# Healthcare-Robotics/mr-gan

Measured on AMD Instinct MI355X. Metric: GAN train steps/sec (labeled+unlabeled+G) at batch 4096, higher is better.
Workload: dtype bf16; 1 GPU; BASELINE configs[1]: synthetic N=65536 x D=512, K=6, batch 4096 per GPU, labeled 100/class; one step = D sub-step (3B rows) + G sub-step (2B rows) + both Adam updates; global_batch=4096, rows_per_gpu=4096, parallelism=single, batch_statistics=n/a, launch=hipGraph replay

## Files before the change

include/mrgan_abi.h:

```cpp
#ifndef MRGAN_ABI_H
#define MRGAN_ABI_H

#include <stddef.h>
#include <stdint.h>

#ifdef __cplusplus
extern "C" {
#endif

typedef struct mrgan_handle mrgan_handle;
typedef void* mrgan_stream;

enum { MRGAN_F32 = 0, MRGAN_BF16 = 1, MRGAN_FP8 = 2 };
enum { MRGAN_NET_G = 0, MRGAN_NET_D = 1 };
enum {
    MRGAN_FLAG_SYNC_STATS = 1,
    MRGAN_FLAG_FLAT_GRADS = 2,
    MRGAN_FLAG_GRAPH      = 4,
    MRGAN_FLAG_GRAD_BF16  = 8,
    MRGAN_FLAG_GAUSS_NOISE = 16
};

#define MRGAN_MAX_CLASSES 32
#define MRGAN_MAX_MODELS 16
// ... 25 lines not shown

int mrgan_select_model(mrgan_handle* h, int model);

int mrgan_num_tensors(const mrgan_handle* h, int net, int* n);
int mrgan_tensor_shape(const mrgan_handle* h, int net, int idx, int* rows, int* cols);
int mrgan_set_weights(mrgan_handle* h, int net, int idx, const float* src_dev, mrgan_stream stream);
int mrgan_get_weights(mrgan_handle* h, int net, int idx, float* dst_dev, mrgan_stream stream);
int mrgan_get_slot(mrgan_handle* h, int net, int idx, int which, float* dst_dev, mrgan_stream stream);
int mrgan_set_slot(mrgan_handle* h, int net, int idx, int which, const float* src_dev, mrgan_stream stream);
int mrgan_get_iterations(mrgan_handle* h, mrgan_stream stream, uint32_t* iterations_host);
int mrgan_set_iterations(mrgan_handle* h, uint32_t iterations, uint32_t batch_counter, mrgan_stream stream);

typedef struct mrgan_disc_args {
    const float* x_lab_dev; const int32_t* idx_lab_dev; const int32_t* labels_dev;
    const float* x_unl_dev; const int32_t* idx_unl_dev;
    const float* z_dev;
    int64_t ld_x_lab, ld_x_unl;
    int32_t stream_mode, reserved;
} mrgan_disc_args;

typedef struct mrgan_gen_args {
    const float* x_unl_dev; const int32_t* idx_unl_dev;
    const float* z_dev;
    int64_t ld_x_unl;
    int32_t stream_mode, reserved;
} mrgan_gen_args;

enum { MRGAN_D_GEN = 0, MRGAN_D_MAIN = 1, MRGAN_D_ADAM = 2, MRGAN_D_NPHASES = 3 };
enum { MRGAN_G_GEN = 0, MRGAN_G_FEAT = 1, MRGAN_G_BWD = 2, MRGAN_G_TAIL = 3, MRGAN_G_ADAM = 4, MRGAN_G_NPHASES = 5 };
int mrgan_disc_step(mrgan_handle* h, const mrgan_disc_args* a, int phase_first, int phase_last,
                    float* out3_host, mrgan_stream stream);
int mrgan_gen_step(mrgan_handle* h, const mrgan_gen_args* a, int phase_first, int phase_last,
                   float* out1_host, mrgan_stream stream);
enum { MRGAN_FP8_DRY_PASSES = 5 };
enum { MRGAN_FP8_CAL_QUERY = 0, MRGAN_FP8_CAL_BEGIN = 1, MRGAN_FP8_CAL_END_PASS = 2, MRGAN_FP8_CAL_DONE = 3 };
int mrgan_fp8_calibration(mrgan_handle* h, int kind, int action, mrgan_stream stream);

typedef struct mrgan_sup_args {
    const float* x_dev; const int32_t* idx_dev; const int32_t* labels_dev;
    int64_t ld_x;
    int32_t stream_mode, rows_valid;
} mrgan_sup_args;
int mrgan_sup_step(mrgan_handle* h, const mrgan_sup_args* a, float* out2_host, mrgan_stream stream);
typedef struct mrgan_sup_group_args {
    const float* x_dev; const int32_t* idx_dev; const int32_t* labels_dev;
    int64_t ld_x;
    int64_t x_model_stride, idx_model_stride, labels_model_stride;
    int32_t stream_mode, rows_valid;
} mrgan_sup_group_args;
int mrgan_sup_step_group(mrgan_handle* h, const mrgan_sup_group_args* a, float* out2_host, mrgan_stream stream);

int32_t mrgan_logmel_frames(int64_t n_samples);
int mrgan_logmel(const float* y_dev, int64_t n_trials, int64_t n_samples, int64_t ld_y, int32_t sr, int32_t n_mels,
                 float* out_dev, int64_t ld_out, mrgan_stream stream);

int mrgan_train_pair(mrgan_handle* h, const mrgan_disc_args* d, const mrgan_gen_args* g, mrgan_stream stream);
int mrgan_pair_hint(mrgan_handle* h, int on);

typedef struct mrgan_disc_group_args {
    const float* x_lab_dev; const int32_t* idx_lab_dev; const int32_t* labels_dev;
    const float* x_unl_dev; const int32_t* idx_unl_dev;
    const float* z_dev;
    int64_t ld_x_lab, ld_x_unl;
    int64_t x_lab_model_stride, idx_lab_model_stride, labels_model_stride;
    int64_t x_unl_model_stride, idx_unl_model_stride, z_model_stride;
    int32_t stream_mode, reserved;
} mrgan_disc_group_args;
typedef struct mrgan_gen_group_args {
    const float* x_unl_dev; const int32_t* idx_unl_dev;
    const float* z_dev;
    int64_t ld_x_unl;
    int64_t x_unl_model_stride, idx_unl_model_stride, z_model_stride;
    int32_t stream_mode, reserved;
} mrgan_gen_group_args;
int mrgan_disc_step_group(mrgan_handle* h, const mrgan_disc_group_args* a, float* out3_host, mrgan_stream stream);
int mrgan_gen_step_group(mrgan_handle* h, const mrgan_gen_group_args* a, float* out1_host, mrgan_stream stream);
int mrgan_train_pair_group(mrgan_handle* h, const mrgan_disc_group_args* d, const mrgan_gen_group_args* g, mrgan_stream stream);

enum {
    MRGAN_TUNE_CHAIN = 0,
    MRGAN_TUNE_KC_CFG = 1,
    MRGAN_TUNE_KS_GROUP = 4,
    MRGAN_TUNE_PAIR_GEN = 5,
    MRGAN_TUNE_HEAD_MFMA = 6
};
int mrgan_set_tuning(mrgan_handle* h, int knob, int value);

enum {
    MRGAN_REGION_BN_STATS = 0,
    MRGAN_REGION_FM_MOMENTS = 1,
    MRGAN_REGION_BN_BWD = 2,
    MRGAN_REGION_GRAD_D = 3,
    MRGAN_REGION_GRAD_G = 4,
    MRGAN_REGION_WORKSPACE = 5,
    MRGAN_REGION_GRAD_D_BF16 = 6,
    MRGAN_REGION_GRAD_G_BF16 = 7,
    MRGAN_REGION_TAIL_D = 8,
    MRGAN_REGION_TAIL_G = 9
};
int mrgan_region(mrgan_handle* h, int region, void** ptr_dev, size_t* bytes);

int mrgan_eval_error(mrgan_handle* h, const float* x_dev, const int32_t* idx_dev, int64_t ld_x,
                     const int32_t* labels_dev, int64_t n, float* err_host, mrgan_stream stream);
int mrgan_predict_logits(mrgan_handle* h, const float* x_dev, const int32_t* idx_dev, int64_t ld_x, int64_t n,
                         float* logits_dev, mrgan_stream stream);

enum { MRGAN_SAL_LOGIT = 0, MRGAN_SAL_XENT = 1, MRGAN_SAL_MSE = 2 };
enum { MRGAN_SAL_RAW = 0, MRGAN_SAL_HEATMAP = 1 };
typedef struct mrgan_saliency_args {
    const float* x_dev; const int32_t* idx_dev; int64_t ld_x; int64_t n;
    const int32_t* targets_dev;
    int32_t objective;
    int32_t post;
    float* out_dev; int64_t ld_out;
    int32_t* classes_out_dev;
} mrgan_saliency_args;
int mrgan_input_gradient(mrgan_handle* h, const mrgan_saliency_args* a, mrgan_stream stream);

enum { MRGAN_ATTR_NOISE = 0, MRGAN_ATTR_PATH = 1 };
enum { MRGAN_ATTR_MAX_DRAWS = 4096, MRGAN_ATTR_NOISE_SEG = 255 };
typedef struct mrgan_attribution_args {
    const float* x_dev; const int32_t* idx_dev; int64_t ld_x; int64_t n;
    const int32_t* targets_dev;
    int32_t objective;
    int32_t post;
    float* out_dev; int64_t ld_out;
    int32_t* classes_out_dev;
    int32_t method;
    int32_t draws;
    float sigma_input, sigma_hidden;
    const float* baseline_dev;
    int32_t multiply;
    int32_t reserved;
} mrgan_attribution_args;
int mrgan_attribution(mrgan_handle* h, const mrgan_attribution_args* a, mrgan_stream stream);

int mrgan_read_metrics(mrgan_handle* h, float* out8_host, int reset, mrgan_stream stream);

enum { MRGAN_PROF_NAME_LEN = 96 };
int mrgan_profile_begin(mrgan_handle* h);
int mrgan_profile_end(mrgan_handle* h, mrgan_stream stream, int max_kernels, char* names, float* ms, int32_t* launches,
                      double* flops, double* bytes, int* n_kernels);

#ifdef __cplusplus
}
#endif
#endif
```

include/mrgan_debug.h:

```cpp
#ifndef MRGAN_DEBUG_H
#define MRGAN_DEBUG_H

#include "mrgan_abi.h"

#ifdef __cplusplus
extern "C" {
#endif

int mrgan_debug_noise(mrgan_handle* h, uint32_t site, uint32_t seg, uint32_t step, uint32_t row0, int rows, int cols,
                      float* out_dev, mrgan_stream stream);
int mrgan_debug_tr_probe(uint16_t* out1024_dev, mrgan_stream stream);
int mrgan_debug_ablate(mrgan_handle* h, int bits);
int mrgan_debug_buffer(mrgan_handle* h, int kind, int l, void** ptr_dev, int* rows_per_seg, int* ld, int* elem_size);
int mrgan_debug_gemm_time(int op, int m, int n, int k, int nbatch, int splits, int reps, int ablate, int kc_cfg, float* avg_us);

typedef struct mrgan_debug_gemm_desc {
    int32_t dtype, op, m, n, k, nbatch, splits;
    int32_t kchunk;
    int32_t kc_cfg;
    int32_t tune_bits;
    int32_t seg_stride, seg_rows;
    const void* a; int64_t a_bs, a_si, a_sk;
    const void* b; int64_t b_bs, b_sk, b_sj;
    int32_t act, n_valid;
    const float* bias;
    void* out; int64_t out_bs; int32_t ldo;
    float sigma; uint32_t site, seg0; int32_t seg_step; uint32_t iter_step, row0;
    uint32_t iter;
    uint64_t seed;
    uint16_t* mask; int64_t mask_bs; int32_t ldm;
    const void* h; int64_t h_bs; int32_t ldh;
    int32_t cs_mode; float* cs1; float* cs2; int32_t ldcs;
    const float* bn_mu; const float* bn_rstd;
    float* slab; int64_t slab_stride;
    void* q8; int64_t q8_bs; int32_t ldq8;
    void* q8t; int64_t q8t_bs; int32_t ldq8t;
    const void* slot_a; const void* slot_b; void* slot_o;
    int32_t gauss;
} mrgan_debug_gemm_desc;
typedef struct mrgan_debug_fold { const float* src; float* dst; int64_t stride; int32_t nsrc, n, ngroups; } mrgan_debug_fold;
int mrgan_debug_gemm_launch(const mrgan_debug_gemm_desc* d, int count, int grouped, const mrgan_debug_fold* fold,
                            char* kname, int kname_len, mrgan_stream stream);

int mrgan_debug_gemm_fp8(int m, int n, int k, const float* a_dev, const float* b_dev, const float* bias_dev, int act, float scale_a,
                         float scale_b, float* out_dev, int reps, float* avg_us, int kc_cfg, mrgan_stream stream);

int mrgan_debug_quant8(const void* src, int64_t src_bs, int ld, int rows, int cols, int nb, int prow, void* dst, int64_t dst_bs, int ldd,
                       void* dstt, int64_t dstt_bs, int lddt, void* slot_dev, int fmt, mrgan_stream stream);
int mrgan_debug_fp8_update_scales(void* slots_dev, int n, mrgan_stream stream);


typedef struct mrgan_debug_stage_seg {
    const float* src; const int32_t* idx; int64_t ld;
    int32_t rows, cols, cols_pad;
    void* out; int32_t ldo;
    float sigma; uint32_t site, seg;
    int32_t gen, stream; uint32_t iter_off;
    int32_t models; int64_t src_ms, idx_ms, out_ms;
} mrgan_debug_stage_seg;
typedef struct mrgan_debug_stage_desc {
    int32_t dtype;
    mrgan_debug_stage_seg s[5]; int32_t nseg;
    uint64_t seed; uint32_t row0;
    uint32_t iter, batch;
    int32_t gauss;
} mrgan_debug_stage_desc;
int mrgan_debug_stage(const mrgan_debug_stage_desc* d, mrgan_stream stream);

int mrgan_debug_reduce_partials(const float* src, int nsrc, int64_t stride, int n, int ngroups, float* dst, int models,
                                int64_t model_stride, mrgan_stream stream);
int mrgan_debug_colsum_finalize(const float* part1, const float* part2, int npart, int ld, int n, float* out, int nseg,
                                mrgan_stream stream);

typedef struct mrgan_debug_bn_apply_desc {
    int32_t dtype;
    const void* h; void* out; int32_t ld, rows, cols;
    const float* cs1; const float* cs2; int32_t npart, ldcs;
    float count, eps;
    const float* gamma; const float* beta;
    float* mu; float* rstd;
    int64_t cs_seg_stride;
    int32_t nseg; int64_t seg_rows;
} mrgan_debug_bn_apply_desc;
int mrgan_debug_bn_apply(const mrgan_debug_bn_apply_desc* d, mrgan_stream stream);

typedef struct mrgan_debug_bn_bwd_desc {
    int32_t dtype;
    const void* dy; const void* h; void* dpre; int32_t ld, rows, cols;
    const float* cs1; const float* cs2; int32_t npart, ldcs;
    float count;
    const float* gamma; const float* mu; const float* rstd;
    float* db_part;
} mrgan_debug_bn_bwd_desc;
int mrgan_debug_bn_bwd(const mrgan_debug_bn_bwd_desc* d, mrgan_stream stream);

typedef struct mrgan_debug_head_desc {
    int32_t dtype;
    const void* f; int64_t f_bs; int32_t ldf;
    int32_t rows, nseg, seg_kind[3];
    int32_t feat, feat_valid, classes;
    const float* w; int32_t ldw; const float* b;
    const int32_t* labels; int32_t labels_stream; uint32_t batch;
    float inv_count, unl_weight;
    float* logits; int64_t logits_bs;
    void* dpre; int64_t dpre_bs; int32_t ldd;
    float* part; int64_t part_stride; int32_t off_db, off_dbf;
    float* loss_part;
    int32_t models; int64_t model_stride, labels_ms;
    int32_t* err_count;
    void* q8; int64_t q8_bs; int32_t ldq8;
    void* q8t; int64_t q8t_bs; int32_t ldq8t;
    void* q8_slot;
} mrgan_debug_head_desc;
int mrgan_debug_head(const mrgan_debug_head_desc* d, mrgan_stream stream);

typedef struct mrgan_debug_head_wide_desc {
    mrgan_debug_head_desc h;
    const uint16_t* mask; int64_t mask_bs; int32_t ldm;
    void* w6c; void* w6r;
} mrgan_debug_head_wide_desc;
int mrgan_debug_head_wide(const mrgan_debug_head_wide_desc* d, mrgan_stream stream);

typedef struct mrgan_debug_fm_desc {
    int32_t dtype;
    const float* cs; int32_t npart_fake, npart_real, ldcs;
    float count, grad_scale; int32_t feat, feat_valid;
    const uint16_t* mask; int32_t ldm;
    void* dpre; int32_t ldd; int32_t rows;
    float* loss_out; float* accum;
    void* q8; int32_t ldq8; void* q8_slot;
    float* lscratch; uint32_t* lcount;
} mrgan_debug_fm_desc;
int mrgan_debug_fm(const mrgan_debug_fm_desc* d, mrgan_stream stream);

typedef struct mrgan_debug_chain_op {
    int32_t K, N, n_valid;
    const void* W; const float* bias;
    float sigma; uint32_t site;
    void* out; int64_t out_bs; int32_t ldo;
    uint16_t* mask; int64_t mask_bs; int32_t ldm;
    float* cs; int32_t ldcs;
} mrgan_debug_chain_op;
typedef struct mrgan_debug_chain_desc {
    int32_t variant;
    mrgan_debug_chain_op fwd[3], dx[3];
    int32_t rows, nseg, block_rows;
    int32_t models; int64_t model_stride;
    const void* a; int64_t a_bs; int32_t lda, a_cols;
    int32_t seg0; uint64_t seed; uint32_t row0; int32_t gauss;
    uint32_t iter, batch;
    mrgan_debug_head_desc head;
    mrgan_debug_fm_desc fm; const void* fm_feat; int32_t fm_ldf;
} mrgan_debug_chain_desc;
int mrgan_debug_chain(const mrgan_debug_chain_desc* d, char* kname, int kname_len, mrgan_stream stream);

typedef struct mrgan_debug_adam_tile {
    float* p; float* m; float* v;
    const float* g; int32_t nslab; int64_t slab_stride;
    float* flat; void* flat16;
    void* w16; void* wt16;
    void* w8; void* w8t; void* w8_slot;
    int32_t ld, ldt, rows, cols;
} mrgan_debug_adam_tile;
typedef struct mrgan_debug_adam_desc {
    const mrgan_debug_adam_tile* tiles; int32_t ntiles, mode;
    float b1, b2, eps;
    uint32_t iter, batch; float lr_t;
    const float* loss_part; int32_t nloss_part; float inv_rows; float* step_out; float* accum;
    float* flat_tail;
    int32_t publish_next, advance_batch; float lr;
    int32_t models; int64_t model_stride;
} mrgan_debug_adam_desc;
int mrgan_debug_adam(const mrgan_debug_adam_desc* d, uint32_t next_out[4], mrgan_stream stream);

#ifdef __cplusplus
}
#endif
// ... 2 lines not shown
```

mr_gan_amd/csrc/aux_kernels.h:

```cpp
#pragma once
#include "common.h"

namespace mrgan {

constexpr int KMAX = 8;
constexpr int KWIDE = 32;
constexpr int class_pitch(int classes) { return classes <= KMAX ? KMAX : KWIDE; }
constexpr int HEAD_ROWS = 32;
constexpr int HEAD_CHUNK = 256;

struct StageSeg {
    const float* src; const int32_t* idx; long ld;
    int rows, cols, cols_pad;
    void* out; int ldo;
    float sigma; uint32_t site, seg;
    int gen;
    int stream;
    uint32_t iter_off;
    int models; long src_ms, idx_ms, out_ms;
};
struct StageArgs {
    StageSeg s[5]; int nseg;
    uint64_t seed; uint32_t row0;
    const DevState* cur;
    int gauss;
    int ry; uint32_t ry_mul;
};
int launch_stage(int bf16, const StageArgs& a, hipStream_t s);

struct BnApplyArgs {
    const void* h; void* out; int ld; int rows; int cols;
    const float* cs1; const float* cs2; int npart; int ldcs;
    float count, eps;
    const float* gamma; const float* beta;
    float* mu; float* rstd;
    long cs_seg_stride;
    int nseg; long seg_rows;
    int models; long model_stride; uint32_t seg_mul;
};
int launch_bn_apply(int bf16, const BnApplyArgs& a, hipStream_t s);

struct BnBwdArgs {
    const void* dy; const void* h; void* dpre; int ld; int rows; int cols;
    const float* cs1; const float* cs2; int npart; int ldcs;
    float count;
    const float* gamma; const float* mu; const float* rstd;
    float* db_part;
    int models; long model_stride;
};
int launch_bn_bwd(int bf16, const BnBwdArgs& a, hipStream_t s);
int stat_row_blocks(int rows);

enum { HEAD_LAB = 0, HEAD_UNL = 1, HEAD_FAKE = 2, HEAD_EVAL = 3, HEAD_LOGITS = 4,
       HEAD_MSE = 5,
       HEAD_SAL_LOGIT = 6, HEAD_SAL_XENT = 7, HEAD_SAL_MSE = 8 };
struct HeadArgs {
    const void* f; long f_bs; int ldf;
    int rows, nseg, seg_kind[3];
    int feat, feat_valid, classes;
    const float* w; int ldw; const float* b;
    const int32_t* labels;
    const DevState* st; int labels_stream;
    float inv_count, unl_weight;
    float* logits; long logits_bs;
    void* dpre; long dpre_bs; int ldd;
    float* part; long part_stride;
    int off_db, off_dbf;
    float* loss_part;
    int models; long model_stride, labels_ms;
    union {
        int* err_count;
        int32_t* classes_out;
    };
    unsigned char* q8; long q8_bs; int ldq8;
    unsigned char* q8t; long q8t_bs; int ldq8t;
    Fp8Slot* q8_slot;
};
int launch_head(int bf16, const HeadArgs& a, hipStream_t s);
int launch_reduce_partials(const float* src, int nsrc, long stride, int n, int ngroups, float* dst, hipStream_t s, int models = 1,
                           long model_stride = 0);
int init_kernel_attributes();

enum { SAL_RAW = 0, SAL_HEATMAP = 1 };
struct SaliencyFinishArgs {
    const void* g; int ldg;
    int rows, cols;
    float* out; long ldo;
    int mode;
};
int launch_saliency_finish(int bf16, const SaliencyFinishArgs& a, hipStream_t s);

struct PathStageArgs {
    const float* src; const int32_t* idx; long ld;
    const float* baseline;
    float alpha;
    int rows, cols, cols_pad;
    void* out; int ldo;
};
int launch_path_stage(int bf16, const PathStageArgs& a, hipStream_t s);
struct AttrAccumArgs {
    const void* g; int ldg;
    int rows, cols;
    float* out; long ldo;
    int mode;
    int draw, draws;
    int multiply;
    const float* x; const int32_t* idx; long ld_x;
    const float* baseline;
};
int launch_attr_accum(int bf16, const AttrAccumArgs& a, hipStream_t s);

struct FmArgs {
    const float* cs; int npart_fake, npart_real, ldcs;
    float count, grad_scale; int feat, feat_valid;
    const uint16_t* mask; int ldm;
    void* dpre; int ldd; int rows;
    float* loss_out; float* accum;
    unsigned char* q8; int ldq8; Fp8Slot* q8_slot;
    int rb;
    float* lscratch; unsigned int* lcount;
    int models; long model_stride;
};
int launch_fm(int bf16, const FmArgs& a, hipStream_t s);

int launch_colsum_finalize(const float* part1, const float* part2, int npart, int ld, int n, float* out , hipStream_t s,
                           int nseg = 1 );

struct AdamTile {
    float* p; float* m; float* v;
    const float* g; int nslab; long slab_stride;
    float* flat;
    __bf16* flat16;
    __bf16* w16; __bf16* wt16;
    unsigned char* w8; unsigned char* w8t; Fp8Slot* w8_slot;
// ... 20 lines not shown
```

mr_gan_amd/csrc/aux_kernels.hip:

```cpp
#include "aux_kernels.h"
#include "head.h"

namespace mrgan {
namespace {

template <typename T> __device__ __forceinline__ void load8(const T* p, float v[8]);
template <> __device__ __forceinline__ void load8<float>(const float* p, float v[8]) {
    const f32x4 a = *(const f32x4*)p, b = *(const f32x4*)(p + 4);
#pragma unroll
    for (int i = 0; i < 4; ++i) { v[i] = a[i]; v[4 + i] = b[i]; }
}
template <> __device__ __forceinline__ void load8<__bf16>(const __bf16* p, float v[8]) {
    const bf16x8 a = *(const bf16x8*)p;
#pragma unroll
    for (int i = 0; i < 8; ++i) v[i] = (float)a[i];
}
template <typename T> __device__ __forceinline__ void store8(T* p, const float v[8]);
template <> __device__ __forceinline__ void store8<float>(float* p, const float v[8]) {
    f32x4 a, b;
#pragma unroll
    for (int i = 0; i < 4; ++i) { a[i] = v[i]; b[i] = v[4 + i]; }
    *(f32x4*)p = a; *(f32x4*)(p + 4) = b;
}
template <> __device__ __forceinline__ void store8<__bf16>(__bf16* p, const float v[8]) {
// ... 21 lines not shown
    const float* const xsrc = sg.src + (long)model * sg.src_ms;
    const int32_t* const xidx = sg.idx ? sg.idx + (long)model * sg.idx_ms : nullptr;
    const bool noisy = sg.gen || sg.sigma > 0.f;
    const float sigs = (sg.gen ? 1.0f : sg.sigma) * (GAUSS ? 1.0f : NOISE_SCALE);
    const int cg = (lane & 15) * 8, rl = lane >> 4;
    const int col = cbase + cg;
    const bool vec_ok = !sg.gen && (sg.ld & 3) == 0 && ((uintptr_t)xsrc & 15) == 0 && col + 7 < sg.cols;
    long srow[8];
#pragma unroll
    for (int it = 0; it < 8; ++it) {
        const int row = rbase + it * 4 + rl;
        srow[it] = (!sg.gen && row < sg.rows) ? (xidx ? (long)xidx[o + row] : (o + row)) : 0;
    }
    float v[8][8];
#pragma unroll
    for (int it = 0; it < 8; ++it) {
#pragma unroll
        for (int c = 0; c < 8; ++c) v[it][c] = 0.f;
        const int row = rbase + it * 4 + rl;
        if (!sg.gen && row < sg.rows) {
            const float* src = xsrc + srow[it] * sg.ld + col;
            if (vec_ok) load8<float>(src, v[it]);
            else {
#pragma unroll
                for (int c = 0; c < 8; ++c) if (col + c < sg.cols) v[it][c] = src[c];
            }
        }
    }
    if constexpr (GAUSS) {
        if (noisy) {
            const uint32_t ph = gauss_pairhash(noise_key(seed, sg.site * 256u + sg.seg, st.iter + sg.iter_off), a.row0 + (uint32_t)rbase, lane);
#pragma unroll
            for (int cb = 0; cb < 4; ++cb) {
                const int c0 = cbase + cb * 32;
                if (c0 >= sg.cols) break;
                const f32x16 nz = gauss_block(ph, (uint32_t)(c0 + lc), lane);
#pragma unroll
                for (int r = 0; r < 16; ++r) glds[wave][acc_row(r, lh)][lc] = nz[r];
                __builtin_amdgcn_fence(__ATOMIC_RELEASE, "wavefront");
                __builtin_amdgcn_wave_barrier();
                if ((cg >> 5) == cb) {
#pragma unroll
                    for (int it = 0; it < 8; ++it) {
                        const f32x4 n0 = *(const f32x4*)&glds[wave][it * 4 + rl][cg & 31], n1 = *(const f32x4*)&glds[wave][it * 4 + rl][(cg & 31) + 4];
#pragma unroll
                        for (int c = 0; c < 4; ++c) {
                            if (col + c < sg.cols) v[it][c] = fmaf(sigs, n0[c], v[it][c]);
                            if (col + 4 + c < sg.cols) v[it][4 + c] = fmaf(sigs, n1[c], v[it][4 + c]);
                        }
                    }
                }
                __builtin_amdgcn_fence(__ATOMIC_ACQ_REL, "wavefront");
                __builtin_amdgcn_wave_barrier();
            }
        }
    } else if (noisy) {
        const uint32_t rowhash = noise_rowhash(noise_key(seed, sg.site * 256u + sg.seg, st.iter + sg.iter_off), a.row0 + (uint32_t)(rbase + lc));
        const i32x4 hfrag = hadamard_frag(lane);
#pragma unroll
        for (int cb = 0; cb < 4; ++cb) {
            const int c0 = cbase + cb * 32;
            if (c0 >= sg.cols) break;
            const i32x16 nz = noise_block(rowhash, (uint32_t)c0 >> 5, lane, hfrag);
#pragma unroll
            for (int r = 0; r < 16; ++r) nlds[wave][acc_row(r, lh)][cb * 32 + lc] = (short)nz[r];
        }
        __builtin_amdgcn_fence(__ATOMIC_RELEASE, "wavefront");
        __builtin_amdgcn_wave_barrier();
    }
    if (col >= sg.cols_pad) return;
#pragma unroll
    for (int it = 0; it < 8; ++it) {
        const int rr = it * 4 + rl, row = rbase + rr;
        if (row >= sg.rows) break;
        if (!GAUSS && noisy && col < sg.cols) {
            const s16x8 nz = *(const s16x8*)&nlds[wave][rr][cg];
#pragma unroll
            for (int c = 0; c < 8; ++c) if (col + c < sg.cols) v[it][c] = fmaf(sigs, (float)nz[c], v[it][c]);
        }
        store8<T>(out + (long)row * sg.ldo + col, v[it]);
    }
}

constexpr int RB = 64, CB = 64;

__device__ __forceinline__ void fold_partials(const float* part, int npart, int ldcs, int col0, int ncols, float (*scr)[CB], float* out) {
    const int t = threadIdx.x, cq = (t & 15) * 4, pl = t >> 4;
    f32x4 s0 = {0.f, 0.f, 0.f, 0.f}, s1 = s0;
    if (col0 + cq < ncols) {
        int p = pl;
        for (; p + 16 < npart; p += 32) {
            s0 += *(const f32x4*)(part + (long)p * ldcs + col0 + cq);
            s1 += *(const f32x4*)(part + (long)(p + 16) * ldcs + col0 + cq);
        }
        for (; p < npart; p += 16) s0 += *(const f32x4*)(part + (long)p * ldcs + col0 + cq);
    }
    s0 += s1;
    *(f32x4*)(&scr[pl][cq]) = s0;
    __syncthreads();
    if (t < CB) {
        float s = 0.f;
#pragma unroll
        for (int k = 0; k < 16; ++k) s += scr[k][t];
        out[t] = s;
    }
    __syncthreads();
}

template <typename T>
__global__ __launch_bounds__(256) void bn_apply_kernel(const BnApplyArgs a) {
    __shared__ float sc[CB], sh[CB];
    __shared__ float scr[16][CB], f1[CB], f2[CB];
    const int t = threadIdx.x, col0 = blockIdx.x * CB;
    const int model = (int)((blockIdx.z * a.seg_mul) >> 16), seg = (int)blockIdx.z - model * a.nseg;
    const long moff = (long)model * a.model_stride;
    const float* const gamma = (const float*)((const char*)a.gamma + moff);
    const float* const beta = (const float*)((const char*)a.beta + moff);
    float* const mu = (float*)((char*)a.mu + moff);
    float* const rstd_out = (float*)((char*)a.rstd + moff);
    fold_partials((const float*)((const char*)a.cs1 + moff) + (long)seg * a.cs_seg_stride, a.npart, a.ldcs, col0, a.ld, scr, f1);
    fold_partials((const float*)((const char*)a.cs2 + moff) + (long)seg * a.cs_seg_stride, a.npart, a.ldcs, col0, a.ld, scr, f2);
    if (t < CB) {
        const int col = col0 + t;
        float scale = 0.f, shift = 0.f;
        if (col < a.ld) {
            const float mean = f1[t] / a.count;
            const float var = fmaxf(f2[t] / a.count - mean * mean, 0.f);
            const float rstd = 1.0f / sqrtf(var + a.eps);
            if (col < a.cols) { scale = gamma[col] * rstd; shift = beta[col] - mean * scale; }
            if (blockIdx.y == 0) { mu[(long)seg * a.ld + col] = mean; rstd_out[(long)seg * a.ld + col] = rstd; }
        }
        sc[t] = scale; sh[t] = shift;
    }
    __syncthreads();
    const int cg = t & 7, rl = t >> 3, c0 = col0 + cg * 8;
    if (c0 >= a.ld) return;
    const T* h = (const T*)((const char*)a.h + moff) + (long)seg * a.seg_rows * a.ld;
    T* out = (T*)((char*)a.out + moff) + (long)seg * a.seg_rows * a.ld;
    const int r1 = min(a.rows, (int)(blockIdx.y + 1) * RB);
    for (int r = blockIdx.y * RB + rl; r < r1; r += 32) {
        float v[8];
        load8<T>(h + (long)r * a.ld + c0, v);
#pragma unroll
        for (int i = 0; i < 8; ++i) v[i] = v[i] * sc[cg * 8 + i] + sh[cg * 8 + i];
        store8<T>(out + (long)r * a.ld + c0, v);
    }
}

template <typename T>
__global__ __launch_bounds__(256) void bn_bwd_kernel(const BnBwdArgs a) {
    __shared__ float cA[CB], cB[CB], cM[CB], cR[CB], cG[CB];
    __shared__ float red[32][CB];
    const int t = threadIdx.x, col0 = blockIdx.x * CB;
    const long moff = (long)blockIdx.z * a.model_stride;
    fold_partials((const float*)((const char*)a.cs1 + moff), a.npart, a.ldcs, col0, a.ld, red, cB);
    fold_partials((const float*)((const char*)a.cs2 + moff), a.npart, a.ldcs, col0, a.ld, red, cG);
    if (t < CB) {
        const int col = col0 + t;
        float g = 0.f, mu = 0.f, rs = 0.f;
        if (col < a.cols) {
            g = ((const float*)((const char*)a.gamma + moff))[col]; mu = ((const float*)((const char*)a.mu + moff))[col];
            rs = ((const float*)((const char*)a.rstd + moff))[col];
        }
        cA[t] = g * rs / a.count; cM[t] = mu; cR[t] = rs;
    }
    __syncthreads();
    const int cg = t & 7, rl = t >> 3, c0 = col0 + cg * 8;
    float acc[8];
#pragma unroll
    for (int i = 0; i < 8; ++i) acc[i] = 0.f;
    if (c0 < a.ld) {
        const T* dy = (const T*)((const char*)a.dy + moff);
        const T* h = (const T*)((const char*)a.h + moff);
        T* dpre = (T*)((char*)a.dpre + moff);
        const int r1 = min(a.rows, (int)(blockIdx.y + 1) * RB);
        for (int r = blockIdx.y * RB + rl; r < r1; r += 32) {
            float hv[8], d[8], o[8];
            load8<T>(h + (long)r * a.ld + c0, hv);
            load8<T>(dy + (long)r * a.ld + c0, d);
#pragma unroll
            for (int i = 0; i < 8; ++i) {
                const int c = cg * 8 + i;
                const float xh = (hv[i] - cM[c]) * cR[c];
                const float dh = cA[c] * (a.count * d[i] - cB[c] - xh * cG[c]);
                o[i] = dh * (-expm1f(-hv[i]));
                acc[i] += o[i];
            }
            store8<T>(dpre + (long)r * a.ld + c0, o);
        }
    }
#pragma unroll
    for (int i = 0; i < 8; ++i) red[rl][cg * 8 + i] = acc[i];
    __syncthreads();
    if (t < CB && col0 + t < a.ld) {
        float s = 0.f;
#pragma unroll
        for (int k = 0; k < 32; ++k) s += red[k][t];
        ((float*)((char*)a.db_part + moff))[(long)blockIdx.y * a.ld + col0 + t] = s;
    }
}

constexpr int HR = HEAD_ROWS;
template <bool WIDE> struct HeadAcc { typedef float type; };
#ifndef MRGAN_HEAD_ACC_F32
template <> struct HeadAcc<true> { typedef double type; };
#endif
__device__ __forceinline__ float head_fma(float a, float b, float c) { return fmaf(a, b, c); }
__device__ __forceinline__ double head_fma(float a, float b, double c) { return fma((double)a, (double)b, c); }
template <typename T, bool Q8 = false, int KP = KMAX, bool SAL = false>
__global__ __launch_bounds__(256) void head_kernel(const HeadArgs a) {
    constexpr int KG = KP / 4;
    typedef typename HeadAcc<(KP > KMAX && sizeof(T) == 2)>::type acc_t;
    extern __shared__ __attribute__((aligned(16))) float hl[];
    const int CH = min(a.feat, HEAD_CHUNK), nch = (a.feat + CH - 1) / CH;
    const int LDF = CH + 8;
    float* f_lds = hl;
    float* w_lds = f_lds + HR * LDF;
    float* dl_lds = w_lds + CH * KP;
    float* red = dl_lds + HR * KP;

    const int t = threadIdx.x, lane = t & 63, wave = t >> 6;
    const int seg = blockIdx.y, kind = a.seg_kind[seg];
    const int row_blk = blockIdx.x * HR;
    const int blk = seg * gridDim.x + blockIdx.x;
    const long moff = (long)blockIdx.z * a.model_stride;
    const T* f = (const T*)((const char*)a.f + moff) + (long)seg * a.f_bs;
    const float* const w6 = (const float*)((const char*)a.w + moff);

    const int cpr = CH / 8;
    auto load_chunk = [&](int c0) {
        for (int ci = t; ci < HR * cpr; ci += 256) {
            const int r = ci / cpr, c = (ci - r * cpr) * 8;
            float v[8] = {0.f, 0.f, 0.f, 0.f, 0.f, 0.f, 0.f, 0.f};
            if (row_blk + r < a.rows && c0 + c < a.feat) load8<T>(f + (long)(row_blk + r) * a.ldf + c0 + c, v);
            *(f32x4*)(f_lds + r * LDF + c) = (f32x4){v[0], v[1], v[2], v[3]};
            *(f32x4*)(f_lds + r * LDF + c + 4) = (f32x4){v[4], v[5], v[6], v[7]};
        }
        for (int k = t; k < CH; k += 256) {
            f32x4 w[KG];
#pragma unroll
            for (int g = 0; g < KG; ++g) w[g] = (f32x4){0.f, 0.f, 0.f, 0.f};
            if (c0 + k < a.feat_valid) {
#pragma unroll
                for (int g = 0; g < KG; ++g) w[g] = *(const f32x4*)(w6 + (long)(c0 + k) * a.ldw + 4 * g);
            }
#pragma unroll
            for (int c = 0; c < 4; ++c)
#pragma unroll
                for (int g = 0; g < KG; ++g) if (c + 4 * g >= a.classes) w[g][c] = 0.f;
#pragma unroll
            for (int g = 0; g < KG; ++g) *(f32x4*)(w_lds + k * KP + 4 * g) = w[g];
        }
    };

    constexpr int LPR = 256 / HR;
    const int r = t / LPR, part = t % LPR;
    acc_t la[KP];
#pragma unroll
    for (int c = 0; c < KP; ++c) la[c] = 0.f;
    for (int ch = 0; ch < nch; ++ch) {
        if (ch) __syncthreads();
        load_chunk(ch * CH);
        __syncthreads();
        for (int kk = 0; kk < CH / LPR; ++kk) {
            const int k = kk * LPR + part;
            const float fv = f_lds[r * LDF + k];
            f32x4 w[KG];
#pragma unroll
            for (int g = 0; g < KG; ++g) w[g] = *(const f32x4*)(w_lds + k * KP + 4 * g);
// ... 756 lines not shown
```

mr_gan_amd/csrc/engine.hip:

```cpp
#include "engine_internal.h"

namespace mrgan {
thread_local LaunchTimer g_launch_timer = {nullptr, nullptr, 0, 0};
}

namespace {

int prof_cat(mrgan_handle* h, const char* name) {
    for (size_t i = 0; i < h->prof_names.size(); ++i)
        if (h->prof_names[i] == name) return (int)i;
    h->prof_names.push_back(name);
    return (int)h->prof_names.size() - 1;
}
__global__ void prof_delay_kernel(int us) {
    for (int i = 0; i < us; ++i) __builtin_amdgcn_s_sleep(36);
}


void prof_backlog(mrgan_handle* h, hipStream_t s) {
    if (!h->prof) return;
    hipLaunchKernelGGL(prof_delay_kernel, dim3(1), dim3(64), 0, s, 400);
}
void prof_arm(mrgan_handle* h) {
    if (!h->prof) return;
// ... 77 lines not shown
              int ldd, unsigned char* dstt, long dstt_bs, int lddt, int slot, int fmt, hipStream_t s) {
    Quant8Args q;
    memset(&q, 0, sizeof q);
    q.src = (const __bf16*)src; q.src_bs = src_bs; q.ld = ld; q.rows = rows; q.cols = cols; q.prow = prow; q.nb = nb;
    q.dst = dst; q.dst_bs = dst_bs; q.ldd = ldd; q.dstt = dstt; q.dstt_bs = dstt_bs; q.lddt = lddt;
    q.slot = h->slots + slot; q.fmt = fmt;
    PROFB("quant8_kernel", launch_quant8(q, s), (double)nb * prow * cols * (2.0 + (dst ? 1.0 : 0.0) + (dstt ? 1.0 : 0.0)));
    return 0;
}
int fp8_quant_images(mrgan_handle* h, const void* src, int width, int nb, unsigned char* img, unsigned char* imgt, int ldt, int slot,
                     int fmt, hipStream_t s) {
    const long bs = (long)h->S * width;
    return fp8_quant(h, src, bs, width, h->B, width, (int)round_up(h->B, 64), nb, img, bs, width, imgt, h->S, ldt, slot, fmt, s);
}

int dense_fwd(mrgan_handle* h, const Dense& L, int kind, const void* x, int rows, int nb, void* out, int act, const NoiseSite& nz,
              const ReluMask& m, const ColSums& cs, hipStream_t s, const Fp8Use& f8 = NO_FP8, const DrawKey* dk = nullptr) {
    const Fp8Images& q = L.q;
    const bool fp8 = q.on && kind != KIND_EVAL;
    const long a_bs = (long)h->S * L.Kp;
    if (fp8 && f8.quant_in)
        CHK(fp8_quant_images(h, x, L.Kp, nb, x8_view(h, L), f8.wgrad ? x8t_view(h, L) : nullptr, q.ldxt, q.sx[kind], FP8_E4M3, s));
    GemmArgs g = with_handle(h, fp8       ? gemm_fwd_args(rows, L.Kp, L.Np, nb, x8_view(h, L), a_bs, L.Kp, q.w8t, L.Kp, true)
                                : h->bf16 ? gemm_fwd_args(rows, L.Kp, L.Np, nb, x, a_bs, L.Kp, L.W->wt16, L.Kp, true)
                                          : gemm_fwd_args(rows, L.Kp, L.Np, nb, x, a_bs, L.Kp, L.W->p, L.Np, false));
    Epi& e = g.e;
    e.act = act; e.n_valid = L.N; e.bias = L.b->p;
    if (kind == KIND_EVAL) {
        e.st = nullptr;
        if (dk) { e.st = dk->st; e.seed = dk->seed; e.row0 = dk->row0; }
        g.B = selected(h, g.B); e.bias = selected(h, e.bias);
    }
    e.out = out; e.out_bs = (long)h->S * L.Np; e.ldo = L.Np;
    e.sigma = nz.sigma; e.site = nz.site; e.seg0 = nz.seg0; e.seg_step = nz.seg_step; e.iter_step = nz.iter_step;
    epi_mask(h, e, m);
    epi_sums(e, cs, L.Np);
    if (fp8) {
        e.qa = h->slots + q.sx[kind]; e.qb = h->slots + q.sw;
        if (f8.to && f8.to->q.on) epi_images(h, e, f8.to->q.x8, f8.wgrad ? f8.to->q.x8t : nullptr, L.Np, f8.to->q.ldxt, f8.to->q.sx[kind]);
    }
    return run_gemm(h, EPI_FWD, g, 2.0 * rows * nb * L.K * L.N, dense_bytes(h, (double)rows * nb, L), s);
}

int dense_dx(mrgan_handle* h, const Dense& L, int kind, const void* dy, int rows, int nb, void* out, int act, int n_valid,
             const ReluMask& m, const void* hprev, const ColSums& cs, hipStream_t s, const Fp8Use& f8 = NO_FP8) {
    const Fp8Images& q = L.q;
    const long a_bs = (long)h->S * L.Np;
    if (q.on && f8.quant_in)
        CHK(fp8_quant_images(h, dy, L.Np, nb, q.g8, f8.wgrad ? q.g8t : nullptr, q.ldgt, q.sg[kind], FP8_E5M2, s));
    GemmArgs g = with_handle(h, q.on ? gemm_dx_args(rows, L.Kp, L.Np, nb, q.g8, a_bs, L.Np, q.w8, L.Np)
                                     : gemm_dx_args(rows, L.Kp, L.Np, nb, dy, a_bs, L.Np,
                                                    h->bf16 ? (const void*)L.W->w16 : (const void*)L.W->p, L.Np));
    Epi& e = g.e;
    e.act = act; e.n_valid = n_valid;
    if (kind == KIND_EVAL) g.B = selected(h, g.B);
    e.out = out; e.out_bs = (long)h->S * L.Kp; e.ldo = L.Kp;
    epi_mask(h, e, m);
    e.h = hprev; e.h_bs = (long)h->S * L.Kp; e.ldh = L.Kp;
    epi_sums(e, cs, L.Kp);
    e.bn_mu = h->bn_mu; e.bn_rstd = h->bn_rstd;
    if (q.on) {
        e.qa = h->slots + q.sg[kind]; e.qb = h->slots + q.sw;
        if (f8.to && f8.to->q.on) epi_images(h, e, f8.to->q.g8, f8.wgrad ? f8.to->q.g8t : nullptr, L.Kp, f8.to->q.ldgt, f8.to->q.sg[kind]);
    }
    return run_gemm(h, EPI_DX, g, 2.0 * rows * nb * L.K * L.N, dense_bytes(h, (double)rows * nb, L), s);
}

double dw_args(mrgan_handle* h, GemmArgs& g, const Dense& L, int kind, const void* x, const void* dy, int rows, int nseg) {
    const bool dense = h->bf16 != 0;
    const int vrows = dense ? nseg * h->S : (nseg - 1) * h->S + rows;
    if (L.q.on) {
        g = with_handle(h, gemm_dw_args(L.Kp, L.Np, vrows, L.splits, vrows / L.splits, 0, 0, x8t_view(h, L), L.q.ldxt, L.q.g8t, L.q.ldgt,
                                        true, L.slabs));
        g.e.qa = h->slots + L.q.sx[kind]; g.e.qb = h->slots + L.q.sg[kind];
    } else {
        g = with_handle(h, gemm_dw_args(L.Kp, L.Np, vrows, L.splits, gemm_dw_kchunk(vrows, L.splits), h->S, dense ? h->S : rows,
                                        x, L.Kp, dy, L.Np, false, L.slabs));
    }
    return 2.0 * rows * nseg * L.K * L.N;
}

struct DwJob { const Dense* L; const void* x; const void* dy; };

int dense_dw_all(mrgan_handle* h, int kind, const DwJob* jobs, int n, int rows, int nseg, hipStream_t s, const FoldJob* fold = nullptr) {
    GemmArgs gs[KS_GROUP_MAX];
    DwJob js[KS_GROUP_MAX];
    double fl[KS_GROUP_MAX], total = 0.0, bytes = 0.0;
    if (n > KS_GROUP_MAX) return fail(-1, "dense_dw_all: too many products");
    std::copy(jobs, jobs + n, js);
    const int ngroup = (int)(std::stable_partition(js, js + n, [](const DwJob& j) { return !j.L->q.on; }) - js);
    for (int i = 0; i < n; ++i) fl[i] = dw_args(h, gs[i], *js[i].L, kind, js[i].x, js[i].dy, rows, nseg);
    for (int i = 0; i < ngroup; ++i) { total += fl[i] * h->grouped; bytes += dw_bytes(h, (double)rows * nseg, *js[i].L) * h->grouped; }
    int first = 0;
    if (h->bf16 && ngroup > 0) {
        const char* kname = "gemm";
        prof_arm(h);
        const int r = launch_gemm_bf16_dw_group(gs, ngroup, s, &kname, fold);
        prof_done(h, kname, total, bytes);
        if (r < 0) return fail(r, "grouped weight-gradient launch failed");
        if (r == 0) { first = ngroup; fold = nullptr; }
    }
    for (int i = first; i < n; ++i) CHK(run_gemm(h, EPI_SLAB, gs[i], fl[i], dw_bytes(h, (double)rows * nseg, *js[i].L), s));
    if (fold) PROF("reduce_partials_kernel", launch_reduce_partials(fold->src, fold->nsrc, fold->stride, fold->n, fold->ngroups, fold->dst, s,
                                                                    h->grouped, fold->model_stride));
    return 0;
}

}
int mrgan::fp8_update_scales(mrgan_handle* h, hipStream_t s) {
    PROF("fp8_update_scales_kernel", launch_fp8_update_scales(h->slots, FP8_NSLOT, s));
    return 0;
}
int mrgan::fp8_refresh_weights(mrgan_handle* h, int net, hipStream_t s) {
    int n;
    const Dense* Ls = net_layers(h, net, &n);
    for (int l = 0; l < n; ++l) {
        const Dense& L = Ls[l];
        if (L.q.on) CHK(fp8_quant(h, L.W->w16, 0, L.Np, L.Kp, L.Np, L.Kp, 1, L.q.w8, 0, L.Np, L.q.w8t, 0, L.Kp, L.q.sw, FP8_E4M3, s));
    }
    return 0;
}
namespace {

int run_adam(mrgan_handle* h, int net, int mode, bool with_metrics, hipStream_t s, int advance_batch = 0) {
    AdamArgs a;
    memset(&a, 0, sizeof a);
    if (mode != ADAM_REDUCE_ONLY) { a.next = h->state + (h->cur ^ 1); a.advance_batch = advance_batch; a.lr = h->cfg.lr; }
    a.tiles = net == MRGAN_NET_D ? h->tiles_d_dev : h->tiles_g_dev;
    a.ntiles = net == MRGAN_NET_D ? h->ntiles_d : h->ntiles_g;
    a.mode = mode; a.b1 = h->cfg.beta1; a.b2 = h->cfg.beta2; a.eps = h->cfg.adam_eps;
    a.st = h->state + h->cur;
    if (with_metrics) {
        a.loss_part = h->loss_part; a.nloss_part = h->head_nblk; a.inv_rows = 1.0f / (float)h->Bg;
        a.step_out = h->step_out; a.accum = h->accum;
        a.flat_tail = h->flat_d + h->flat_d_n;
    }
    a.models = h->grouped; a.model_stride = (long)h->W;
    {
        const std::vector<Tensor>& ts = net == MRGAN_NET_D ? h->dt : h->gt;
        double bytes = 0.0;
        for (const Tensor& t : ts) bytes += (double)t.prow * t.pcol * (24.0 + 4.0 * std::max(1, t.nslab) + (t.w16 ? 4.0 : 0.0));
        PROFB("adam_kernel", launch_adam(a, s), bytes);
    }
    return 0;
}

int gen_fwd_head(mrgan_handle* h, int nb, hipStream_t s) {
    CHK(dense_fwd(h, h->g[0], KIND_D, h->zbuf, h->B, nb, h->h1, ACT_SOFTPLUS, NO_NOISE, NO_MASK, ColSums{CS_SUM_SQ, h->cs_bn1, h->cs_bn2}, s));
    if (h->sync_stats) {
        const int n = h->g[0].Np;
        PROF("colsum_finalize_kernel", launch_colsum_finalize(h->cs_bn1, h->cs_bn2, h->tiles_m, n, n, h->r_bn_stats, s, nb));
    }
    return 0;
}
int gen_fwd_tail(mrgan_handle* h, int nb, int fake_seg_slot, uint32_t fake_seg_id, hipStream_t s) {
    const int n = h->g[0].Np;
    BnApplyArgs b;
    memset(&b, 0, sizeof b);
    b.h = h->h1; b.out = h->hbn; b.ld = n; b.rows = h->B; b.cols = h->g[0].N;
    b.nseg = nb; b.seg_rows = h->S;
    if (h->sync_stats) { b.cs1 = h->r_bn_stats; b.cs2 = h->r_bn_stats + n; b.npart = 1; b.cs_seg_stride = 2 * n; }
    else { b.cs1 = h->cs_bn1; b.cs2 = h->cs_bn2; b.npart = h->tiles_m; b.cs_seg_stride = (long)h->tiles_m * n; }
    b.ldcs = n; b.count = h->stat_count; b.eps = h->cfg.bn_eps;
    b.gamma = h->gt[2].p; b.beta = h->gt[3].p; b.mu = h->bn_mu; b.rstd = h->bn_rstd;
    b.models = h->grouped; b.model_stride = (long)h->W;
    PROF("bn_apply_kernel", launch_bn_apply(h->bf16, b, s));
    CHK(dense_fwd(h, h->g[1], KIND_D, h->hbn, h->B, nb, h->h2, ACT_SOFTPLUS, NO_NOISE, NO_MASK, NO_SUMS, s, Fp8Use{nullptr, true, true}));
    void* out = rowptr(h, h->xin[0], (long)fake_seg_slot * h->S, h->Dp);
    const NoiseSite nz = {h->cfg.sigma[0], 0, fake_seg_id, nb > 1 ? -(int)fake_seg_id : 1, nb > 1 ? 1u : 0u};
    CHK(dense_fwd(h, h->g[2], KIND_D, h->h2, h->B, nb, out, ACT_LINEAR, nz, NO_MASK, NO_SUMS, s));
    return 0;
}

int disc_fwd_train(mrgan_handle* h, int kind, int nb, bool fm_sums, int x0_slot, hipStream_t s, int l_end = 5) {
    for (int l = 0; l < l_end; ++l) {
        const void* in = l == 0 ? rowptr(h, h->xin[0], (long)x0_slot * h->S, h->Dp) : h->xin[l];
        void* out = l < 4 ? h->xin[l + 1] : h->feat;
        const NoiseSite nz = {l < 4 ? h->cfg.sigma[l + 1] : 0.f, (uint32_t)(l + 1), 0, 1, 0};
        const bool last = l == 4;
        CHK(dense_fwd(h, h->d[l], kind, in, h->B, nb, out, ACT_RELU, nz, relu_mask(h, l), ColSums{(last && fm_sums) ? CS_SUM : CS_NONE, h->cs_f, nullptr},
                      s, Fp8Use{last ? nullptr : &h->d[l + 1], kind == KIND_D, l == 0}));
    }
// ... 212 lines not shown

int gen_chain_fwd(mrgan_handle* h, hipStream_t s) {
    ChainArgs c = chain_args(h, CH_V_GFWD, 2, chain_block_rows(h, 2));
    for (int i = 0; i < 3; ++i) c.fwd[i] = chain_fwd_op(h, 2 + i, i == 2);
    return run_chain(h, c, chain_flops(h, c, false), s);
}

int fm_grad(mrgan_handle* h, hipStream_t s) {
    FmArgs f;
    memset(&f, 0, sizeof f);
    if (h->sync_stats) { f.cs = h->r_fm; f.npart_fake = 1; f.npart_real = 1; }
    else { f.cs = h->cs_f; f.npart_fake = f.npart_real = fm_parts(h); }
    f.ldcs = h->Fp; f.count = h->stat_count; f.grad_scale = h->fm_scale; f.feat = h->Fp; f.feat_valid = h->F;
    f.mask = h->mask[4]; f.ldm = h->ldm[4]; f.dpre = h->dpre[4]; f.ldd = h->Fp; f.rows = h->B;
    f.loss_out = h->step_out + 3; f.accum = h->accum + 3;
    f.lscratch = h->fm_scratch; f.lcount = h->fm_count;
    f.models = h->grouped; f.model_stride = (long)h->W;
    if (h->fp8) { f.dpre = nullptr; f.q8 = h->d[4].q.g8; f.ldq8 = h->Fp; f.q8_slot = h->slots + h->d[4].q.sg[KIND_G]; }
    if (!h->use_chain) {
        PROF("fm_kernel", launch_fm(h->bf16, f, s));
        return 0;
    }
    ChainArgs c = chain_args(h, CH_V_GBWD, 1, chain_block_rows(h, 1));
    c.fm = f; c.fm_feat = (const __bf16*)h->feat; c.fm_ldf = h->Fp;
    for (int i = 0; i < 3; ++i) c.dx[i] = chain_dx_op(h, 4 - i, false);
    return run_chain(h, c, chain_flops(h, c, false), s);
}

int disc_dx_to_input(mrgan_handle* h, hipStream_t s) {
    for (int l = h->use_chain ? 1 : 4; l >= 1; --l)
        CHK(dense_dx(h, h->d[l], KIND_G, h->dpre[l], h->B, 1, h->dpre[l - 1], ACT_RELU, h->d[l - 1].N, relu_mask(h, l - 1), nullptr,
                     NO_SUMS, s, Fp8Use{&h->d[l - 1], false, false}));
    return dense_dx(h, h->d[0], KIND_G, h->dpre[0], h->B, 1, h->dxfake, ACT_LINEAR, h->cfg.d_in, NO_MASK, nullptr,
                    ColSums{CS_SUM, h->cs_db3g, nullptr}, s);
}

int gen_phase(mrgan_handle* h, const mrgan_gen_args* a, int phase, hipStream_t s) {
    const int B = h->B, tm = h->tiles_m, N1p = h->g[0].Np;
    if (phase == MRGAN_G_GEN) {
        prof_backlog(h, s);
        StageArgs st;
        memset(&st, 0, sizeof st);
        const bool ready = h->gen_ready && !a->z_dev;
        h->gen_ready = ready ? 1 : 0;
        h->xbase = ready ? 3 : 0;
        set_gen_view(h, ready ? 1 : 0);
        const bool staged = ready && h->real_staged;
        h->real_staged = 0;
        if (!staged) {
            data_seg(st.s[0], h, a->x_unl_dev, a->idx_unl_dev, a->ld_x_unl, h->xbase + 1, 1, a->stream_mode, h->gs.x_unl, h->gs.idx_unl);
            st.nseg = 1;
            stage_common(st, h, a->z_dev, a->stream_mode, ready ? -1 : 1);
            PROF("stage_kernel", launch_stage(h->bf16, st, s));
        }
        if (!ready) CHK(gen_fwd_head(h, 1, s));
    } else if (phase == MRGAN_G_FEAT) {
        if (!h->gen_ready) CHK(gen_fwd_tail(h, 1, 0, 0, s));
        h->gen_ready = 0;
        CHK(disc_fwd_train(h, 1, 2, true, h->xbase, s, h->use_chain ? 2 : 5));
        if (h->use_chain) CHK(gen_chain_fwd(h, s));
        if (h->sync_stats) {
            const int np = fm_parts(h);
            PROF("colsum_finalize_kernel", launch_colsum_finalize(h->cs_f, h->cs_f + (size_t)np * h->Fp, np, h->Fp, h->Fp, h->r_fm, s));
        }
    } else if (phase == MRGAN_G_BWD) {
        CHK(fm_grad(h, s));
        CHK(disc_dx_to_input(h, s));
        CHK(dense_dx(h, h->g[2], KIND_G, h->dxfake, B, 1, h->dpre2g, ACT_SOFTPLUS, h->g[1].N, NO_MASK, h->h2,
                     ColSums{CS_SUM, h->cs_db2g, nullptr}, s));
        CHK(dense_dx(h, h->g[1], KIND_G, h->dpre2g, B, 1, h->dhbn, ACT_LINEAR, h->g[0].N, NO_MASK, h->h1,
                     ColSums{CS_SUM_XHAT, h->cs_dbeta, h->cs_dgamma}, s, Fp8Use{nullptr, true, true}));
        if (h->sync_stats) {
            PROF("colsum_finalize_kernel", launch_colsum_finalize(h->cs_dbeta, h->cs_dgamma, tm, N1p, N1p, h->r_bn_bwd, s));
        }
    } else if (phase == MRGAN_G_TAIL) {
        BnBwdArgs b;
        memset(&b, 0, sizeof b);
        b.dy = h->dhbn; b.h = h->h1; b.dpre = h->dpre1g; b.ld = N1p; b.rows = B; b.cols = h->g[0].N;
        if (h->sync_stats) { b.cs1 = h->r_bn_bwd; b.cs2 = h->r_bn_bwd + N1p; b.npart = 1; }
        else { b.cs1 = h->cs_dbeta; b.cs2 = h->cs_dgamma; b.npart = tm; }
        b.ldcs = N1p; b.count = h->stat_count; b.gamma = h->gt[2].p; b.mu = h->bn_mu; b.rstd = h->bn_rstd;
        b.db_part = h->db1g_part;
        b.models = h->grouped; b.model_stride = (long)h->W;
        PROF("bn_bwd_kernel", launch_bn_bwd(h->bf16, b, s));
        const DwJob jobs[3] = {{&h->g[2], h->h2, h->dxfake}, {&h->g[0], h->zbuf, h->dpre1g}, {&h->g[1], h->hbn, h->dpre2g}};
        CHK(dense_dw_all(h, KIND_G, jobs, 3, B, 1, s));
        if (h->flat_grads) CHK(run_adam(h, MRGAN_NET_G, ADAM_REDUCE_ONLY, false, s));
    } else if (phase == MRGAN_G_ADAM) {
        CHK(run_adam(h, MRGAN_NET_G, h->flat_grads ? ADAM_FROM_FLAT : ADAM_FUSED, false, s, a->stream_mode ? 1 : 0));
        if (h->fp8) CHK(fp8_update_scales(h, s));
        h->cur ^= 1;
    }
    return 0;
}

int sup_step(mrgan_handle* h, const mrgan_sup_args* a, hipStream_t s) {
    const int B = h->B;
    prof_backlog(h, s);
    StageArgs st;
    memset(&st, 0, sizeof st);
    data_seg(st.s[0], h, a->x_dev, a->idx_dev, a->ld_x, 0, 0, a->stream_mode, h->gs.x_lab, h->gs.idx_lab);
    st.nseg = 1;
    stage_common(st, h, nullptr, 0, -1);
    PROF("stage_kernel", launch_stage(h->bf16, st, s));
    CHK(disc_fwd_train(h, 0, 1, false, 0, s, 5));
    HeadArgs hd = head_args(h, {HEAD_MSE}, B, true);
    hd.labels = a->labels_dev; hd.labels_stream = a->stream_mode;
    hd.inv_count = 1.0f / (float)(a->rows_valid > 0 ? a->rows_valid : B); hd.unl_weight = 0.f;
    PROF("head_kernel", launch_head(h->bf16, hd, s));
    h->head_nblk = 3 * ceil_div(B, HEAD_ROWS);
    CHK(disc_bwd(h, 1, 4, ceil_div(B, HEAD_ROWS), s));
    CHK(run_adam(h, MRGAN_NET_D, ADAM_FUSED, true, s, a->stream_mode ? 1 : 0));
    h->cur ^= 1;
    return 0;
}

int check_disc_args(const mrgan_handle* h, const mrgan_disc_args* a) {
    if (!a || !a->x_lab_dev || !a->x_unl_dev || !a->labels_dev) return fail(-2, "disc_step: x_lab, x_unl and labels are required");
    if (a->ld_x_lab < h->cfg.d_in || a->ld_x_unl < h->cfg.d_in) return fail(-2, "disc_step: row pitch smaller than d_in");
    return 0;
}
int check_gen_args(const mrgan_handle* h, const mrgan_gen_args* a) {
    if (!a || !a->x_unl_dev) return fail(-2, "gen_step: x_unl is required");
    if (a->ld_x_unl < h->cfg.d_in) return fail(-2, "gen_step: row pitch smaller than d_in");
    return 0;
}
int check_sup_args(const mrgan_handle* h, const mrgan_sup_args& a, const char* entry) {
    if (a.ld_x < h->cfg.d_in) return fail(-2, "%s: row pitch smaller than d_in", entry);
    if (h->flat_grads || h->cfg.world != 1) return fail(-3, "%s: single-GPU handles only", entry);
    if (h->fp8) return fail(-3, "%s: the fp8 mode covers the GAN step only", entry);
    if (a.rows_valid < 0 || a.rows_valid > h->B) return fail(-2, "%s: rows_valid outside [0, batch]", entry);
    if (a.rows_valid && a.stream_mode) return fail(-2, "%s: a short batch cannot be combined with stream mode", entry);
    return 0;
}

struct GroupScope {
    mrgan_handle* h;
    GroupScope(mrgan_handle* h_, const mrgan_handle::GroupStrides& gs) : h(h_) { h->grouped = h->models; h->gs = gs; h->pair_gen = 0; h->pair_g = nullptr; }
    ~GroupScope() { h->grouped = 1; memset(&h->gs, 0, sizeof h->gs); }
};
mrgan_disc_args single_args(const mrgan_disc_group_args* a) {
    mrgan_disc_args d;
    memset(&d, 0, sizeof d);
    d.x_lab_dev = a->x_lab_dev; d.idx_lab_dev = a->idx_lab_dev; d.labels_dev = a->labels_dev;
    d.x_unl_dev = a->x_unl_dev; d.idx_unl_dev = a->idx_unl_dev; d.z_dev = a->z_dev;
    d.ld_x_lab = a->ld_x_lab; d.ld_x_unl = a->ld_x_unl; d.stream_mode = a->stream_mode;
    return d;
}
mrgan_gen_args single_args(const mrgan_gen_group_args* a) {
    mrgan_gen_args g;
    memset(&g, 0, sizeof g);
    g.x_unl_dev = a->x_unl_dev; g.idx_unl_dev = a->idx_unl_dev; g.z_dev = a->z_dev; g.ld_x_unl = a->ld_x_unl; g.stream_mode = a->stream_mode;
    return g;
}
mrgan_sup_args single_args(const mrgan_sup_group_args* a) {
    mrgan_sup_args u;
    memset(&u, 0, sizeof u);
    u.x_dev = a->x_dev; u.idx_dev = a->idx_dev; u.labels_dev = a->labels_dev; u.ld_x = a->ld_x;
    u.stream_mode = a->stream_mode; u.rows_valid = a->rows_valid;
    return u;
}
int sup_step_group(mrgan_handle* h, const mrgan_sup_group_args* a, hipStream_t s) {
    GroupScope scope(h, {(long)a->x_model_stride, (long)a->idx_model_stride, (long)a->labels_model_stride, 0, 0, 0});
    const mrgan_sup_args u = single_args(a);
    return sup_step(h, &u, s);
}
int disc_step_group(mrgan_handle* h, const mrgan_disc_group_args* a, hipStream_t s) {
    GroupScope scope(h, {(long)a->x_lab_model_stride, (long)a->idx_lab_model_stride, (long)a->labels_model_stride,
                         (long)a->x_unl_model_stride, (long)a->idx_unl_model_stride, (long)a->z_model_stride});
// ... 479 lines not shown
```

mr_gan_amd/csrc/engine_debug.hip:

```cpp
#include "engine_internal.h"

namespace mrgan {
int launch_tr_probe(unsigned short* out, hipStream_t s);
}

namespace {

template <typename T>
__global__ void to_f32_kernel(const T* src, long lds, float* dst, long ldd, int rows, int cols) {
    const int c = blockIdx.x * 64 + (threadIdx.x & 63), r = blockIdx.y * 4 + (threadIdx.x >> 6);
    if (r >= rows || c >= cols) return;
    dst[(long)r * ldd + c] = Elem<T>::to_f32(src[(long)r * lds + c]);
}

}

extern "C" {

int mrgan_debug_noise(mrgan_handle* h, uint32_t site, uint32_t seg, uint32_t step, uint32_t row0, int rows, int cols, float* out,
                      mrgan_stream stream) {
    if (!h || !out) return fail(-1, "null argument");
    if (h->gauss && (row0 & 1u)) return fail(-1, "debug_noise: a true-Gaussian handle draws row pairs, row0 must be even");
    CHK(launch_noise_debug(h->gauss, h->cfg.seed, site, seg, step, row0, rows, cols, out, (hipStream_t)stream));
    return 0;
// ... 309 lines not shown
}

int mrgan_debug_stage(const mrgan_debug_stage_desc* d, mrgan_stream stream) {
    if (!d || d->nseg < 1 || d->nseg > 5) return fail(-1, "debug_stage: 1 .. 5 segments");
    if (d->dtype != MRGAN_F32 && d->dtype != MRGAN_BF16) return fail(-1, "debug_stage: dtype must be fp32 or bf16");
    if (d->gauss && (d->row0 & 1u)) return fail(-1, "debug_stage: the true-Gaussian generator draws row pairs, row0 must be even");
    StageArgs a;
    memset(&a, 0, sizeof a);
    for (int i = 0; i < d->nseg; ++i) {
        const mrgan_debug_stage_seg& g = d->s[i];
        StageSeg& o = a.s[i];
        if (!g.out || g.rows < 1 || g.cols < 1 || (!g.gen && !g.src)) return fail(-1, "debug_stage: segment %d: null argument", i);
        if (g.cols_pad < g.cols || (g.cols_pad % 8) || g.ldo < g.cols_pad || (g.ldo % 8) || !al(g.out, 16) || (g.out_ms % 16))
            return fail(-1, "debug_stage: segment %d: rows of out are stored 8 elements at a time (out, out_ms, ldo %% 8, cols <= cols_pad <= ldo, cols_pad %% 8)", i);
        if (!g.gen && g.ld < g.cols) return fail(-1, "debug_stage: segment %d: ld >= cols", i);
        o.src = g.src; o.idx = g.idx; o.ld = g.ld; o.rows = g.rows; o.cols = g.cols; o.cols_pad = g.cols_pad;
        o.out = g.out; o.ldo = g.ldo; o.sigma = g.sigma; o.site = g.site; o.seg = g.seg; o.gen = g.gen; o.stream = g.stream;
        o.iter_off = g.iter_off; o.models = g.models; o.src_ms = g.src_ms; o.idx_ms = g.idx_ms; o.out_ms = g.out_ms;
    }
    a.nseg = d->nseg; a.seed = d->seed; a.row0 = d->row0; a.gauss = d->gauss;
    DevState* st = nullptr;
    if (int r = debug_devstate(d->iter, d->batch, 0.f, &st)) return r;
    a.cur = st;
    hipStream_t s = (hipStream_t)stream;
    const int r = debug_finish("debug_stage", launch_stage(d->dtype == MRGAN_BF16, a, s), s);
    hipFree(st);
    return r;
}

int mrgan_debug_reduce_partials(const float* src, int nsrc, int64_t stride, int n, int ngroups, float* dst, int models, int64_t model_stride,
                                mrgan_stream stream) {
    if (!src || !dst || nsrc < 1 || n < 1 || ngroups < 1 || models < 1) return fail(-1, "debug_reduce_partials: empty problem");
    if (stride < n) return fail(-1, "debug_reduce_partials: stride >= n");
    if (model_stride % 4) return fail(-1, "debug_reduce_partials: model_stride counts bytes of whole floats");
    hipStream_t s = (hipStream_t)stream;
    return debug_finish("debug_reduce_partials", launch_reduce_partials(src, nsrc, stride, n, ngroups, dst, s, models, model_stride), s);
}

int mrgan_debug_colsum_finalize(const float* part1, const float* part2, int npart, int ld, int n, float* out, int nseg, mrgan_stream stream) {
    if (!part1 || !part2 || !out || npart < 1 || n < 1 || nseg < 1) return fail(-1, "debug_colsum_finalize: empty problem");
    if (!al(part1, 16) || !al(part2, 16) || (ld % 4)) return fail(-1, "debug_colsum_finalize: partial rows are read 16 bytes at a time (pointers, ld %% 4)");
    if (ld < n) return fail(-1, "debug_colsum_finalize: ld >= n");
    hipStream_t s = (hipStream_t)stream;
    return debug_finish("debug_colsum_finalize", launch_colsum_finalize(part1, part2, npart, ld, n, out, s, nseg), s);
}

static int debug_cs_check(const char* who, const float* cs1, const float* cs2, int npart, int ldcs, int width) {
    if (!cs1 || !cs2 || npart < 1) return fail(-1, "%s: column partial sums missing", who);
    if (!al(cs1, 16) || !al(cs2, 16) || (ldcs % 4)) return fail(-1, "%s: partial sums are read 16 bytes at a time (pointers, ldcs %% 4)", who);
    if (ldcs < width) return fail(-1, "%s: ldcs must hold the %d columns the kernel folds", who, width);
    return 0;
}

int mrgan_debug_bn_apply(const mrgan_debug_bn_apply_desc* d, mrgan_stream stream) {
    if (!d || !d->h || !d->out || !d->gamma || !d->beta || !d->mu || !d->rstd || d->rows < 1 || d->cols < 1) return fail(-1, "debug_bn_apply: null argument");
    if (d->dtype != MRGAN_F32 && d->dtype != MRGAN_BF16) return fail(-1, "debug_bn_apply: dtype must be fp32 or bf16");
    if (int r = debug_cs_check("debug_bn_apply", d->cs1, d->cs2, d->npart, d->ldcs, d->ld)) return r;
    if (d->ld < d->cols || (d->ld % 8) || !al(d->h, 16) || !al(d->out, 16)) return fail(-1, "debug_bn_apply: ld >= cols, ld %% 8 == 0 and 16-byte aligned h / out");
    if (d->nseg > 1 && ((d->cs_seg_stride % 4) || d->seg_rows < d->rows)) return fail(-1, "debug_bn_apply: cs_seg_stride %% 4 == 0 and seg_rows >= rows");
    BnApplyArgs a;
    memset(&a, 0, sizeof a);
    a.h = d->h; a.out = d->out; a.ld = d->ld; a.rows = d->rows; a.cols = d->cols;
    a.cs1 = d->cs1; a.cs2 = d->cs2; a.npart = d->npart; a.ldcs = d->ldcs; a.count = d->count; a.eps = d->eps;
    a.gamma = d->gamma; a.beta = d->beta; a.mu = d->mu; a.rstd = d->rstd;
    a.cs_seg_stride = d->cs_seg_stride; a.nseg = d->nseg; a.seg_rows = d->seg_rows;
    hipStream_t s = (hipStream_t)stream;
    return debug_finish("debug_bn_apply", launch_bn_apply(d->dtype == MRGAN_BF16, a, s), s);
}

int mrgan_debug_bn_bwd(const mrgan_debug_bn_bwd_desc* d, mrgan_stream stream) {
    if (!d || !d->dy || !d->h || !d->dpre || !d->gamma || !d->mu || !d->rstd || !d->db_part || d->rows < 1 || d->cols < 1) return fail(-1, "debug_bn_bwd: null argument");
    if (d->dtype != MRGAN_F32 && d->dtype != MRGAN_BF16) return fail(-1, "debug_bn_bwd: dtype must be fp32 or bf16");
    if (int r = debug_cs_check("debug_bn_bwd", d->cs1, d->cs2, d->npart, d->ldcs, d->ld)) return r;
    if (d->ld < d->cols || (d->ld % 8) || !al(d->h, 16) || !al(d->dy, 16) || !al(d->dpre, 16)) return fail(-1, "debug_bn_bwd: ld >= cols, ld %% 8 == 0 and 16-byte aligned dy / h / dpre");
    BnBwdArgs a;
    memset(&a, 0, sizeof a);
    a.dy = d->dy; a.h = d->h; a.dpre = d->dpre; a.ld = d->ld; a.rows = d->rows; a.cols = d->cols;
    a.cs1 = d->cs1; a.cs2 = d->cs2; a.npart = d->npart; a.ldcs = d->ldcs; a.count = d->count;
    a.gamma = d->gamma; a.mu = d->mu; a.rstd = d->rstd; a.db_part = d->db_part;
    hipStream_t s = (hipStream_t)stream;
    return debug_finish("debug_bn_bwd", launch_bn_bwd(d->dtype == MRGAN_BF16, a, s), s);
}

int mrgan_debug_head(const mrgan_debug_head_desc* d, mrgan_stream stream) {
    if (!d || !d->f || !d->w || !d->b || d->rows < 1 || d->nseg < 1 || d->nseg > 3 || d->feat < 1 || d->classes < 1) return fail(-1, "debug_head: null argument");
    if (d->dtype != MRGAN_F32 && d->dtype != MRGAN_BF16) return fail(-1, "debug_head: dtype must be fp32 or bf16");
    const int es = d->dtype == MRGAN_BF16 ? 2 : 4, kp = d->ldw;
    bool losses = false, labels = false;
    for (int i = 0; i < d->nseg; ++i) {
        const int k = d->seg_kind[i];
        if (k < HEAD_LAB || k > HEAD_MSE) return fail(-1, "debug_head: unknown segment kind %d", k);
        losses |= k != HEAD_EVAL && k != HEAD_LOGITS;
        labels |= k == HEAD_LAB || k == HEAD_EVAL || k == HEAD_MSE;
    }
    if (d->feat_valid < 0 || d->feat_valid > d->feat || d->ldf < d->feat) return fail(-1, "debug_head: feat_valid <= feat <= ldf");
    if (!al(d->f, 16) || ((int64_t)d->ldf * es % 16) || (d->f_bs * es % 16)) return fail(-1, "debug_head: feature rows are read 16 bytes at a time (f, ldf, f_bs)");
    if (!al(d->w, 16)) return fail(-1, "debug_head: w must be 16-byte aligned");
    if (labels && !d->labels) return fail(-1, "debug_head: the segment kinds need labels");
    if (losses && !d->loss_part) return fail(-1, "debug_head: training kinds need loss_part");
    if (losses && (!d->part || !al(d->part, 16) || (d->part_stride % 4) || (d->off_db % 4) || d->off_db < (int64_t)d->feat * kp || d->off_dbf < d->off_db + kp ||
                  d->part_stride < (int64_t)d->off_dbf + d->feat))
        return fail(-1, "debug_head: part rows hold dW6 [feat * ldw), db6 at off_db, the bias gradient at off_dbf, 16-byte aligned");
    if (d->dpre && d->ldd < d->feat) return fail(-1, "debug_head: ldd >= feat");
    if (d->models > 1 && (d->model_stride % 16)) return fail(-1, "debug_head: model_stride must keep the 16-byte alignments");
    if (d->q8_slot) {
        if (d->q8 && (!al(d->q8, 4) || (d->ldq8 % 4) || (d->q8_bs % 4) || d->ldq8 < d->feat)) return fail(-1, "debug_head: q8 is stored 4 bytes at a time, ldq8 >= feat");
        if (d->q8t && (!al(d->q8t, 16) || (d->ldq8t % 16) || (d->q8t_bs % 16) || d->q8t_bs < 0 ||
                       d->ldq8t < (int64_t)(d->nseg - 1) * d->q8t_bs + round_up(d->rows, HEAD_ROWS)))
            return fail(-1, "debug_head: q8t is stored 16 bytes at a time and holds nseg segments of round_up(rows, 32) bytes");
    }
    DevState* st = nullptr;
    if (int r = debug_devstate(0, d->batch, 0.f, &st)) return r;
    HeadArgs a;
    debug_head_args(d, st, a);
    hipStream_t s = (hipStream_t)stream;
    static int attr = init_kernel_attributes();
    int r = attr;
    if (!r) r = launch_head(d->dtype == MRGAN_BF16, a, s);
    r = debug_finish("debug_head", r, s);
    hipFree(st);
    return r;
}

static void debug_head_args(const mrgan_debug_head_desc* d, const DevState* st, HeadArgs& a) {
    memset(&a, 0, sizeof a);
    a.f = d->f; a.f_bs = d->f_bs; a.ldf = d->ldf; a.rows = d->rows; a.nseg = d->nseg;
    for (int i = 0; i < 3; ++i) a.seg_kind[i] = d->seg_kind[i];
    a.feat = d->feat; a.feat_valid = d->feat_valid; a.classes = d->classes;
    a.w = d->w; a.ldw = d->ldw; a.b = d->b; a.labels = d->labels; a.st = st; a.labels_stream = d->labels_stream;
    a.inv_count = d->inv_count; a.unl_weight = d->unl_weight;
    a.logits = d->logits; a.logits_bs = d->logits_bs; a.dpre = d->dpre; a.dpre_bs = d->dpre_bs; a.ldd = d->ldd;
    a.part = d->part; a.part_stride = d->part_stride; a.off_db = d->off_db; a.off_dbf = d->off_dbf; a.loss_part = d->loss_part;
    a.models = d->models; a.model_stride = d->model_stride; a.labels_ms = d->labels_ms; a.err_count = d->err_count;
    a.q8 = (unsigned char*)d->q8; a.q8_bs = d->q8_bs; a.ldq8 = d->ldq8;
    a.q8t = (unsigned char*)d->q8t; a.q8t_bs = d->q8t_bs; a.ldq8t = d->ldq8t; a.q8_slot = (Fp8Slot*)d->q8_slot;
}

int mrgan_debug_head_wide(const mrgan_debug_head_wide_desc* w, mrgan_stream stream) {
    if (!w || !w->h.f || !w->h.w || !w->h.b || w->h.rows < 1 || w->h.nseg < 1 || w->h.nseg > 3 || w->h.feat < 1 || w->h.classes < 1)
        return fail(-1, "debug_head_wide: null argument");
    const mrgan_debug_head_desc* d = &w->h;
    const int kp = d->ldw;
    if (d->models > 1) return fail(-1, "debug_head_wide: one model");
    if (d->feat_valid < 0 || d->feat_valid > d->feat || d->ldf < d->feat) return fail(-1, "debug_head_wide: feat_valid <= feat <= ldf");
    if (!al(d->f, 16) || (d->ldf % 8) || (d->f_bs % 8)) return fail(-1, "debug_head_wide: feature rows are read 16 bytes at a time (f, ldf, f_bs)");
    if (w->w6c && w->w6r && (!al(w->w6c, 16) || !al(w->w6r, 16))) return fail(-1, "debug_head_wide: w6c / w6r must be 16-byte aligned");
    if (w->mask && w->ldm < d->feat) return fail(-1, "debug_head_wide: ldm >= feat");
    if (!d->labels) return fail(-1, "debug_head_wide: labels");
    if (d->part && (!al(d->part, 16) || (d->part_stride % 4) || (d->off_db % 4) || d->off_db < (int64_t)d->feat * kp || d->off_dbf < d->off_db + kp ||
                    d->part_stride < (int64_t)d->off_dbf + d->feat))
        return fail(-1, "debug_head_wide: part rows hold dW6 [feat * ldw), db6 at off_db, the bias gradient at off_dbf, 16-byte aligned");
    if (d->dpre && (!al(d->dpre, 16) || (d->ldd % 8) || (d->dpre_bs % 8) || d->ldd < d->feat)) return fail(-1, "debug_head_wide: dpre is stored 16 bytes at a time, ldd >= feat");
    if (d->q8_slot) {
        if (d->q8 && (!al(d->q8, 16) || (d->ldq8 % 16) || (d->q8_bs % 16) || d->ldq8 < d->feat)) return fail(-1, "debug_head_wide: q8 is stored 16 bytes at a time, ldq8 >= feat");
        if (d->q8t && (!al(d->q8t, 16) || (d->ldq8t % 16) || (d->q8t_bs % 16) || d->q8t_bs < 0 ||
                       d->ldq8t < (int64_t)(d->nseg - 1) * d->q8t_bs + round_up(d->rows, HEAD_WIDE_ROWS)))
            return fail(-1, "debug_head_wide: q8t is stored 16 bytes at a time and holds nseg segments of round_up(rows, 64) bytes");
    }
    DevState* st = nullptr;
    if (int r = debug_devstate(0, d->batch, 0.f, &st)) return r;
    HeadWideArgs a;
    debug_head_args(d, st, a.h);
    a.mask = w->mask; a.mask_bs = w->mask_bs; a.ldm = w->ldm; a.w6c = (__bf16*)w->w6c; a.w6r = (__bf16*)w->w6r;
    hipStream_t s = (hipStream_t)stream;
    static int attr = head_wide_init_attributes();
    int r = attr;
// ... 157 lines not shown
```

mr_gan_amd/csrc/engine_internal.h:

```cpp
#pragma once
#include <math.h>
#include <stdio.h>
#include <string.h>

#include <algorithm>
#include <string>
#include <vector>

#include "../../include/mrgan_abi.h"
#include "../../include/mrgan_debug.h"
#include "aux_kernels.h"
#include "chain.h"
#include "head_wide.h"
#include "logmel.h"
#include "gemm.h"

namespace mrgan {

int fail(int code, const char* fmt, ...);
#define HIPCHK(x)                                                                               \
    do {                                                                                        \
        hipError_t e_ = (x);                                                                    \
        if (e_ != hipSuccess) return fail(-10, "%s failed: %s", #x, hipGetErrorString(e_));     \
    } while (0)
// ... 6 lines not shown
constexpr int SEG_ALIGN = 128;

struct Dense;
struct Tensor {
    int rows, cols;
    int prow, pcol;
    float *p, *m, *v;
    __bf16 *w16, *wt16;
    float* flat;
    __bf16* flat16;
    const float* g; int nslab; long slab_stride;
    const Dense* layer;
};

struct Fp8Images {
    bool on;
    unsigned char *x8, *x8t; int ldxt;
    unsigned char *g8, *g8t; int ldgt;
    unsigned char *w8, *w8t;
    int xseg;
    int sx[2], sg[2], sw;
};

struct Dense {
    int K, N, Kp, Np, act;
    Tensor *W, *b;
    float* slabs; int splits;
    Fp8Images q;
};

struct ProfRec { int cat; hipEvent_t start, stop; double flops, bytes; };

constexpr int FP8_NSLOT = 28, FP8_DRY_PASSES = MRGAN_FP8_DRY_PASSES;
constexpr float FP8_TARGET_E4M3 = 224.0f, FP8_TARGET_E5M2 = 28672.0f;


}

using namespace mrgan;

struct mrgan_handle {
    mrgan_config cfg;
    bool bf16, sync_stats, flat_grads, own_ws;
    int gauss;
    int es;
    int B, S, tiles_m, Bg;
    float stat_count, fm_scale;
    int Dp, nzp, Fp, F;
    char* ws; size_t ws_bytes;
    int models;
    size_t W;
    int sel;
    int grouped;
    struct GroupStrides { long x_lab, idx_lab, labels, x_unl, idx_unl, z; } gs;

    std::vector<Tensor> gt, dt;
    Dense g[3], d[6];

    DevState* state;
    DevState* draw_state = nullptr;
    ~mrgan_handle() { if (draw_state) hipFree(draw_state); }
    int cur;
    float* step_out;
    float* accum;
    int* err_count;
    float *flat_d, *flat_g; size_t flat_d_n, flat_g_n;
    __bf16 *flat16_d, *flat16_g;
    float *r_bn_stats, *r_fm, *r_bn_bwd;

    void *zbuf, *h1, *hbn, *h2;
    void *zbuf_all, *h1_all, *hbn_all, *h2_all;
    int pair_gen, gen_ready;
    const mrgan_gen_args* pair_g; int real_staged;
    int xbase;
    void* xin[5]; void* feat; uint16_t* mask[5]; int ldm[5];
    void* dpre[5];
    void *dxfake, *dpre2g, *dhbn, *dpre1g;
    float* logits;
    float *bn_mu, *bn_rstd, *bn_mu_all, *bn_rstd_all;
    float *cs_bn1, *cs_bn2, *cs_db[4], *cs_f, *cs_db3g, *cs_db2g, *cs_dbeta, *cs_dgamma, *db1g_part;
    float *head_part, *head_red, *loss_part; int head_stride, head_groups;
    int head_nblk;
    int bnb_blocks;
    bool fp8; int fp8_cal[2];
    Fp8Slot* slots; float* slot_targets; float* accum_save;
    float* fm_scratch; unsigned int* fm_count;
    int KP;
    bool chain_ok, use_chain;
    bool dtail_chain() const { return use_chain && KP == KMAX; }
    bool head_wide_ok, head_wide; __bf16 *w6c, *w6r;
    int tune_kc_cfg, tune_bits, tune_pair_gen;
    int ablate;
    AdamTile *tiles_g_dev, *tiles_d_dev; int ntiles_g, ntiles_d;

    bool prof; std::vector<ProfRec> prof_recs; std::vector<std::string> prof_names;

    hipGraphExec_t graph_exec; bool graph_ready; int graph_cur;
    unsigned char graph_key[sizeof(mrgan_disc_group_args) + sizeof(mrgan_gen_group_args)]; size_t graph_key_d, graph_key_g;
};

namespace mrgan {

template <typename P> inline P* model_at(const mrgan_handle* h, P* p, int m) { return p ? (P*)((char*)p + (size_t)m * h->W) : p; }
template <typename P> inline P* selected(const mrgan_handle* h, P* p) { return model_at(h, p, h->sel); }
inline void* rowptr(mrgan_handle* h, void* base, long row, int ld) { return (char*)base + (size_t)row * ld * h->es; }
inline Dense* net_layers(mrgan_handle* h, int net, int* n) { *n = net == MRGAN_NET_G ? 3 : 6; return net == MRGAN_NET_G ? h->g : h->d; }
inline dim3 grid2d(int prow, int pcol) { return dim3(ceil_div(pcol, 64), ceil_div(prow, 4)); }
void set_gen_view(mrgan_handle* h, int seg);
int fp8_refresh_weights(mrgan_handle* h, int net, hipStream_t s);
int fp8_update_scales(mrgan_handle* h, hipStream_t s);

}
```

mr_gan_amd/csrc/engine_state.hip:

```cpp
#include <stdarg.h>

#include "engine_internal.h"

namespace mrgan {

thread_local std::string g_err;
int fail(int code, const char* fmt, ...) {
    char buf[512];
    va_list ap;
    va_start(ap, fmt);
    vsnprintf(buf, sizeof buf, fmt, ap);
    va_end(ap);
    g_err = buf;
    return code;
}

void set_gen_view(mrgan_handle* h, int seg) {
    h->g[1].q.xseg = seg;
    const int N1p = h->g[0].Np;
    h->zbuf = rowptr(h, h->zbuf_all, (long)seg * h->S, h->nzp);
    h->h1 = rowptr(h, h->h1_all, (long)seg * h->S, N1p);
    h->hbn = rowptr(h, h->hbn_all, (long)seg * h->S, N1p);
    h->h2 = rowptr(h, h->h2_all, (long)seg * h->S, h->g[1].Np);
    h->bn_mu = h->bn_mu_all + (size_t)seg * N1p;
// ... 141 lines not shown
        h->dt[2 * l].layer = &h->d[l];
    }
    const bool g16 = (c.flags & MRGAN_FLAG_GRAD_BF16) != 0;
    auto flat = [&](std::vector<Tensor>& ts, float*& buf, __bf16*& buf16, size_t& n) {
        n = 0;
        for (auto& t : ts) n += (size_t)t.prow * t.pcol;
        buf = a.take<float>(n + 4);
        buf16 = g16 ? a.take<__bf16>(n) : nullptr;
        size_t o = 0;
        for (auto& t : ts) { t.flat = buf ? buf + o : nullptr; t.flat16 = buf16 ? buf16 + o : nullptr; o += (size_t)t.prow * t.pcol; }
    };
    flat(h->gt, h->flat_g, h->flat16_g, h->flat_g_n);
    flat(h->dt, h->flat_d, h->flat16_d, h->flat_d_n);
    const int N1p = h->g[0].Np;
    h->r_bn_stats = a.take<float>(4 * N1p);
    h->r_fm = a.take<float>(2 * h->Fp);
    h->r_bn_bwd = a.take<float>(2 * N1p);
    h->bn_mu_all = a.take<float>(2 * N1p);
    h->bn_rstd_all = a.take<float>(2 * N1p);

    const size_t es = h->es;
    auto act = [&](size_t rows, size_t cols) { return (void*)a.take<char>(rows * cols * es); };
    h->zbuf_all = act(2 * (size_t)S, h->nzp);
    h->h1_all = act(2 * (size_t)S, N1p); h->hbn_all = act(2 * (size_t)S, N1p); h->h2_all = act(2 * (size_t)S, h->g[1].Np);
    for (int l = 0; l < 5; ++l) {
        h->xin[l] = act((l == 0 ? 5 : 3) * (size_t)S, h->d[l].Kp);
        h->ldm[l] = h->d[l].Np;
        h->mask[l] = a.take<uint16_t>(3 * (size_t)(S / 32) * h->ldm[l] * 2);
        h->dpre[l] = act(3 * (size_t)S, h->d[l].Np);
    }
    h->feat = act(3 * (size_t)S, h->Fp);
    if (h->fp8) {
        auto images = [&](Dense& L, int xseg, int gseg, int sx0, int sx1, int sg0, int sg1, int sw) {
            Fp8Images& q = L.q;
            q.on = true; q.xseg = 0;
            q.ldxt = xseg * S; q.ldgt = gseg * S;
            q.x8 = a.take<unsigned char>((size_t)q.ldxt * L.Kp); q.x8t = a.take<unsigned char>((size_t)q.ldxt * L.Kp);
            q.g8 = a.take<unsigned char>((size_t)q.ldgt * L.Np); q.g8t = a.take<unsigned char>((size_t)q.ldgt * L.Np);
            q.w8 = a.take<unsigned char>((size_t)L.Kp * L.Np); q.w8t = a.take<unsigned char>((size_t)L.Kp * L.Np);
            q.sx[0] = sx0; q.sx[1] = sx1; q.sg[0] = sg0; q.sg[1] = sg1; q.sw = sw;
        };
        for (int l = 0; l < 5; ++l) images(h->d[l], 3, 3, l, 10 + l, 5 + l, 15 + l, 20 + l);
        images(h->g[1], 2, 1, 25, 25, 26, 26, 27);
        h->slots = a.take<Fp8Slot>(FP8_NSLOT); h->slot_targets = a.take<float>(FP8_NSLOT); h->accum_save = a.take<float>(4);
    }
    h->dxfake = act(S, h->Dp); h->dpre2g = act(S, h->g[1].Np); h->dhbn = act(S, N1p); h->dpre1g = act(S, N1p);
    h->logits = a.take<float>(3 * (size_t)S * KP);
    h->fm_scratch = a.take<float>(ceil_div(h->Fp, 64)); h->fm_count = a.take<unsigned int>(4);

    h->cs_bn1 = a.take<float>(2 * (size_t)tm * N1p); h->cs_bn2 = a.take<float>(2 * (size_t)tm * N1p);
    for (int l = 0; l < 4; ++l) h->cs_db[l] = a.take<float>(3 * (size_t)tm * h->d[l].Np);
    h->cs_f = a.take<float>(2 * (size_t)ceil_div(B, 32) * h->Fp);
    h->cs_db3g = a.take<float>((size_t)tm * h->Dp);
    h->cs_db2g = a.take<float>((size_t)tm * h->g[1].Np);
    h->cs_dbeta = a.take<float>((size_t)tm * N1p); h->cs_dgamma = a.take<float>((size_t)tm * N1p);
    h->bnb_blocks = stat_row_blocks(B);
    h->db1g_part = a.take<float>((size_t)h->bnb_blocks * N1p);
    h->chain_ok = h->bf16 && !h->fp8 && h->d[2].Kp <= CH_KMAX && h->d[2].Np <= CH_PW && h->d[3].Np <= CH_PW && h->d[4].Np <= CH_PW &&
                  std::min(std::min(h->d[2].Kp, h->d[2].Np), std::min(h->d[3].Np, h->d[4].Np)) >= 128;
    h->use_chain = h->chain_ok;
    h->head_wide_ok = h->head_wide = h->bf16 && (h->Fp > CH_PW || (KP > KMAX && h->Fp == CH_PW)) && (h->Fp % CH_PW) == 0;
    h->w6c = h->w6r = nullptr;
    if (h->head_wide) { h->w6c = a.take<__bf16>((size_t)3 * KP * h->Fp); h->w6r = a.take<__bf16>((size_t)3 * KP * h->Fp); }
    const int head_cap = 3 * ceil_div(B, HEAD_ROWS);
    h->head_stride = (int)round_up(h->Fp * KP + KP + h->Fp, 64);
    h->head_groups = std::min(8, 3 * ceil_div(B, CH_ROWS));
    h->head_part = a.take<float>((size_t)head_cap * h->head_stride);
    h->head_red = a.take<float>((size_t)h->head_groups * h->head_stride);
    h->loss_part = a.take<float>((size_t)head_cap * 4);

    int tiles_d = 0, tiles_g = 0;
    for (int l = 0; l < 5; ++l) tiles_d += dw_tiles(h->d[l]);
    for (int l = 0; l < 3; ++l) tiles_g += dw_tiles(h->g[l]);
    const int splits_d = choose_splits(tiles_d, 2 * S + B), splits_g = choose_splits(tiles_g, B);
    for (int l = 0; l < 5; ++l) {
        Dense& L = h->d[l];
        L.splits = h->fp8 ? fp8_dw_splits(dw_tiles(L), 3 * S) : splits_d;
        L.slabs = a.take<float>((size_t)L.splits * L.Kp * L.Np);
    }
    for (int l = 0; l < 3; ++l) {
        Dense& L = h->g[l];
        L.splits = (h->fp8 && l == 1) ? 1 : splits_g;
        L.slabs = a.take<float>((size_t)L.splits * L.Kp * L.Np);
    }
    auto src = [&](Tensor& t, const float* g, int nslab, long stride) { t.g = g; t.nslab = nslab; t.slab_stride = stride; };
    for (int l = 0; l < 5; ++l) src(*h->d[l].W, h->d[l].slabs, h->d[l].splits, (long)h->d[l].Kp * h->d[l].Np);
    for (int l = 0; l < 4; ++l) src(*h->d[l].b, h->cs_db[l], 3 * tm, h->d[l].Np);
    src(*h->d[4].b, h->head_red + h->Fp * KP + KP, h->head_groups, h->head_stride);
    src(*h->d[5].W, h->head_red, h->head_groups, h->head_stride);
    src(*h->d[5].b, h->head_red + h->Fp * KP, h->head_groups, h->head_stride);
    for (int l = 0; l < 3; ++l) src(*h->g[l].W, h->g[l].slabs, h->g[l].splits, (long)h->g[l].Kp * h->g[l].Np);
    src(*h->g[0].b, h->db1g_part, h->bnb_blocks, N1p);
    src(h->gt[2], h->cs_dgamma, tm, N1p);
    src(h->gt[3], h->cs_dbeta, tm, N1p);
    src(*h->g[1].b, h->cs_db2g, tm, h->g[1].Np);
    src(*h->g[2].b, h->cs_db3g, tm, h->Dp);

    h->ntiles_g = count_adam_tiles(h->gt); h->ntiles_d = count_adam_tiles(h->dt);
    h->tiles_g_dev = a.take<AdamTile>(h->ntiles_g);
    h->tiles_d_dev = a.take<AdamTile>(h->ntiles_d);

    *bytes_out = (a.off + 255) & ~(size_t)255;
    return 0;
}

int layout(mrgan_handle* h, char* base, size_t* bytes_out) {
    size_t one = 0;
    const int r = layout_model(h, base, &one);
    h->models = std::max(1, (int)h->cfg.models);
    h->W = h->models > 1 ? one : 0;
    *bytes_out = one * (size_t)h->models;
    return r;
}

int upload_tiles(mrgan_handle* h, std::vector<Tensor>& ts, AdamTile* dev, int n, hipStream_t s) {
    std::vector<AdamTile> v;
    const int TR = adam_tile_rows(ts);
    for (auto& t : ts)
        for (int r0 = 0; r0 < t.prow; r0 += TR)
            for (int c0 = 0; c0 < t.pcol; c0 += 64) {
                AdamTile a;
                const long off = (long)r0 * t.pcol + c0;
                a.p = t.p + off; a.m = t.m + off; a.v = t.v + off;
                a.g = t.g + off; a.nslab = t.nslab; a.slab_stride = t.slab_stride;
                a.flat = t.flat + off; a.flat16 = t.flat16 ? t.flat16 + off : nullptr;
                a.w16 = t.w16 ? t.w16 + off : nullptr;
                a.wt16 = t.wt16 ? t.wt16 + (long)c0 * t.prow + r0 : nullptr;
                a.w8 = a.w8t = nullptr; a.w8_slot = nullptr;
                if (t.layer && t.layer->q.on) {
                    const Fp8Images& q = t.layer->q;
                    a.w8 = q.w8 + off; a.w8t = q.w8t + (long)c0 * t.prow + r0; a.w8_slot = h->slots + q.sw;
                }
                a.ld = t.pcol; a.ldt = t.prow;
                a.rows = std::min(TR, t.prow - r0); a.cols = std::min(64, t.pcol - c0);
                v.push_back(a);
            }
    if ((int)v.size() != n) return fail(-20, "tile count mismatch");
    HIPCHK(hipMemcpyAsync(dev, v.data(), sizeof(AdamTile) * n, hipMemcpyHostToDevice, s));
    HIPCHK(hipStreamSynchronize(s));
    return 0;
}

Tensor* find_tensor(mrgan_handle* h, int net, int idx) {
    std::vector<Tensor>& ts = net == MRGAN_NET_G ? h->gt : h->dt;
    if (net != MRGAN_NET_G && net != MRGAN_NET_D) return nullptr;
    if (idx < 0 || idx >= (int)ts.size()) return nullptr;
    return &ts[idx];
}

}

extern "C" {

const char* mrgan_last_error(void) { return g_err.c_str(); }

int mrgan_default_config(mrgan_config* c, int32_t d_in, int32_t batch) {
    if (!c) return fail(-1, "null config");
    memset(c, 0, sizeof *c);
    c->d_in = d_in; c->batch = batch; c->noise_size = 100;
    c->g_hidden[0] = 500; c->g_hidden[1] = 500;
    const int dh[5] = {1000, 500, 250, 250, 250};
    const float sg[5] = {0.3f, 0.5f, 0.5f, 0.5f, 0.5f};
    for (int i = 0; i < 5; ++i) { c->d_hidden[i] = dh[i]; c->sigma[i] = sg[i]; }
    c->num_classes = 6; c->dtype = MRGAN_F32;
    c->lr = 0.0006f; c->beta1 = 0.5f; c->beta2 = 0.999f; c->adam_eps = 1e-8f; c->bn_eps = 2e-5f;
    c->unlabeled_weight = 1.0f; c->seed = 0x5EED5EEDULL; c->rank = 0; c->world = 1; c->flags = 0;
// ... 93 lines not shown
}

int mrgan_tensor_shape(const mrgan_handle* h, int net, int idx, int* rows, int* cols) {
    Tensor* t = find_tensor((mrgan_handle*)h, net, idx);
    if (!t) return fail(-1, "no such tensor (%d,%d)", net, idx);
    *rows = t->rows; *cols = t->cols;
    return 0;
}

int mrgan_select_model(mrgan_handle* h, int model) {
    if (!h) return fail(-1, "null handle");
    if (model < 0 || model >= h->models) return fail(-1, "select_model: model %d outside [0,%d)", model, h->models);
    h->sel = model;
    return 0;
}

int mrgan_set_weights(mrgan_handle* h, int net, int idx, const float* src, mrgan_stream stream) {
    Tensor* t = find_tensor(h, net, idx);
    if (!t || !src) return fail(-1, "set_weights: bad tensor or null source");
    hipStream_t s = (hipStream_t)stream;
    HIPCHK(hipMemcpy2DAsync(selected(h, t->p), sizeof(float) * t->pcol, src, sizeof(float) * t->cols, sizeof(float) * t->cols, t->rows,
                            hipMemcpyDeviceToDevice, s));
    if (t->w16) hipLaunchKernelGGL(refresh_bf16_kernel, grid2d(t->prow, t->pcol), dim3(256), 0, s, selected(h, t->p), selected(h, t->w16), selected(h, t->wt16), t->prow, t->pcol);
    if (t->layer && t->layer->q.on) {
        for (int pass = 0; pass < 2; ++pass) { CHK(fp8_refresh_weights(h, net, s)); CHK(fp8_update_scales(h, s)); }
    }
    return 0;
}

int mrgan_get_weights(mrgan_handle* h, int net, int idx, float* dst, mrgan_stream stream) {
    Tensor* t = find_tensor(h, net, idx);
    if (!t || !dst) return fail(-1, "get_weights: bad tensor or null destination");
    HIPCHK(hipMemcpy2DAsync(dst, sizeof(float) * t->cols, selected(h, t->p), sizeof(float) * t->pcol, sizeof(float) * t->cols, t->rows,
                            hipMemcpyDeviceToDevice, (hipStream_t)stream));
    return 0;
}

int mrgan_get_slot(mrgan_handle* h, int net, int idx, int which, float* dst, mrgan_stream stream) {
    Tensor* t = find_tensor(h, net, idx);
    if (!t || !dst || which < 0 || which > 2) return fail(-1, "get_slot: bad argument");
    if (which == 2 && t->flat16) return fail(-3, "get_slot: the flat gradients of this handle are bfloat16 (MRGAN_REGION_GRAD_*_BF16)");
    const float* src = selected(h, which == 0 ? t->m : which == 1 ? t->v : t->flat);
    HIPCHK(hipMemcpy2DAsync(dst, sizeof(float) * t->cols, src, sizeof(float) * t->pcol, sizeof(float) * t->cols, t->rows,
                            hipMemcpyDeviceToDevice, (hipStream_t)stream));
    return 0;
}

int mrgan_set_slot(mrgan_handle* h, int net, int idx, int which, const float* src, mrgan_stream stream) {
    Tensor* t = find_tensor(h, net, idx);
    if (!t || !src || which < 0 || which > 1) return fail(-1, "set_slot: bad argument");
    float* dst = selected(h, which == 0 ? t->m : t->v);
    HIPCHK(hipMemcpy2DAsync(dst, sizeof(float) * t->pcol, src, sizeof(float) * t->cols, sizeof(float) * t->cols, t->rows,
                            hipMemcpyDeviceToDevice, (hipStream_t)stream));
    return 0;
}

int mrgan_get_iterations(mrgan_handle* h, mrgan_stream stream, uint32_t* it) {
    if (!h || !it) return fail(-1, "null argument");
    DevState st;
    HIPCHK(hipMemcpyAsync(&st, h->state + h->cur, sizeof st, hipMemcpyDeviceToHost, (hipStream_t)stream));
    HIPCHK(hipStreamSynchronize((hipStream_t)stream));
    *it = st.iter;
    return 0;
}

int mrgan_set_iterations(mrgan_handle* h, uint32_t iterations, uint32_t batch_counter, mrgan_stream stream) {
    if (!h) return fail(-1, "null handle");
    hipLaunchKernelGGL(init_state_kernel, dim3(1), dim3(1), 0, (hipStream_t)stream, h->state, iterations, batch_counter,
                       h->cfg.lr, h->cfg.beta1, h->cfg.beta2);
    return 0;
}

int mrgan_set_tuning(mrgan_handle* h, int knob, int value) {
    if (!h) return fail(-1, "null handle");
    if (h->graph_exec) { hipGraphExecDestroy(h->graph_exec); h->graph_exec = nullptr; h->graph_ready = false; }
    switch (knob) {
        case MRGAN_TUNE_CHAIN: h->use_chain = value != 0 && h->chain_ok; break;
        case MRGAN_TUNE_KC_CFG:
            if (!kc_cfg_supported(value)) return fail(-1, "unsupported forward / dX tile config %d", value);
            h->tune_kc_cfg = value; break;
        case MRGAN_TUNE_KS_GROUP: h->tune_bits = (h->tune_bits & ~TUNE_BIT_NO_KS_GROUP) | (value ? 0 : TUNE_BIT_NO_KS_GROUP); break;
        case MRGAN_TUNE_PAIR_GEN: h->tune_pair_gen = value ? 1 : 0; break;
        case MRGAN_TUNE_HEAD_MFMA: h->head_wide = value != 0 && h->head_wide_ok; break;
        default: return fail(-1, "unknown tuning knob %d", knob);
    }
    return 0;
}

int mrgan_pair_hint(mrgan_handle* h, int on) {
    if (!h) return fail(-1, "null handle");
    h->pair_gen = on ? 1 : 0;
    return 0;
}

int mrgan_region(mrgan_handle* h, int region, void** ptr, size_t* bytes) {
    if (!h || !ptr || !bytes) return fail(-1, "null argument");
    const size_t n1 = (size_t)h->g[0].Np;
    switch (region) {
        case MRGAN_REGION_BN_STATS: *ptr = h->r_bn_stats; *bytes = 4 * n1 * 4; break;
        case MRGAN_REGION_FM_MOMENTS: *ptr = h->r_fm; *bytes = 2 * (size_t)h->Fp * 4; break;
        case MRGAN_REGION_BN_BWD: *ptr = h->r_bn_bwd; *bytes = 2 * n1 * 4; break;
        case MRGAN_REGION_GRAD_D: case MRGAN_REGION_GRAD_G: {
            if (h->flat16_d) return fail(-3, "region %d: the gradients of this handle travel as bfloat16 (MRGAN_FLAG_GRAD_BF16): "
                                             "all-reduce MRGAN_REGION_GRAD_*_BF16 and MRGAN_REGION_TAIL_*", region);
            const bool d = region == MRGAN_REGION_GRAD_D;
            *ptr = d ? h->flat_d : h->flat_g; *bytes = ((d ? h->flat_d_n : h->flat_g_n) + 4) * 4;
            break;
        }
        case MRGAN_REGION_WORKSPACE: *ptr = h->ws; *bytes = h->ws_bytes; break;
        case MRGAN_REGION_GRAD_D_BF16: case MRGAN_REGION_GRAD_G_BF16: {
            if (!h->flat16_d) return fail(-3, "the bfloat16 gradient regions exist with MRGAN_FLAG_GRAD_BF16 only");
            const bool d = region == MRGAN_REGION_GRAD_D_BF16;
            *ptr = d ? h->flat16_d : h->flat16_g; *bytes = (d ? h->flat_d_n : h->flat_g_n) * 2;
            break;
        }
        case MRGAN_REGION_TAIL_D: *ptr = h->flat_d + h->flat_d_n; *bytes = 16; break;
        case MRGAN_REGION_TAIL_G: *ptr = h->flat_g + h->flat_g_n; *bytes = 16; break;
        default: return fail(-1, "unknown region %d", region);
    }
    return 0;
}

int mrgan_read_metrics(mrgan_handle* h, float* out8, int reset, mrgan_stream stream) {
    if (!h || !out8) return fail(-1, "null argument");
    hipStream_t s = (hipStream_t)stream;
    HIPCHK(hipMemcpyAsync(out8, selected(h, h->accum), 4 * sizeof(float), hipMemcpyDeviceToHost, s));
    HIPCHK(hipMemcpyAsync(out8 + 4, selected(h, h->step_out), 4 * sizeof(float), hipMemcpyDeviceToHost, s));
    if (reset) HIPCHK(hipMemsetAsync(selected(h, h->accum), 0, 4 * sizeof(float), s));
    HIPCHK(hipStreamSynchronize(s));
    return 0;
}

}
```

mr_gan_amd/csrc/gemm.h:

```cpp
#pragma once
#include <string.h>

#include <algorithm>

#include "common.h"

namespace mrgan {

enum { EPI_FWD = 0, EPI_DX = 1, EPI_SLAB = 2 };
enum { VAR_ACT_MASK = 3, VAR_NOISE = 4, VAR_MASK = 8, VAR_GAUSS = 16, VAR_DYN = 64 };


struct Epi {
    int act;
    int n_valid;
    const float* bias;
    void* out; long out_bs; int ldo;
    float sigma; uint32_t site; uint32_t seg0;
    int seg_step; uint32_t iter_step;
    uint32_t row0;
    uint64_t seed;
    int gauss;
    uint16_t* mask; long mask_bs; int ldm;
    const void* h; long h_bs; int ldh;
// ... 288 lines not shown
            }
        } else if (e.cs_mode != CS_NONE) {
            constexpr int NH = MR >= 2 ? MR / 2 : 1, MH = MR >= 2 ? 2 : 1;
            float cs1[NH][NR], cs2[NH][NR];
#pragma unroll
            for (int hh = 0; hh < NH; ++hh)
#pragma unroll
                for (int ni = 0; ni < NR; ++ni) {
                    const int col = col_blk + (wn * NR + ni) * 32 + lc;
                    float s1 = 0.f, s2 = 0.f;
#pragma unroll
                    for (int m2 = 0; m2 < MH; ++m2) {
                        const int mi = hh * MH + m2;
                        const int rsub = row_blk + (wm * MR + mi) * 32 + 4 * lh;
                        if (e.cs_mode == CS_SUM_XHAT) {
                            const bool cok = col < e.n_valid && col < g.N;
                            const float mu = pf ? pf->mu[ni] : (cok ? model_ptr(e.bn_mu, e, model)[col] : 0.f);
                            const float rstd = pf ? pf->rstd[ni] : (cok ? model_ptr(e.bn_rstd, e, model)[col] : 0.f);
#pragma unroll
                            for (int r = 0; r < 16; ++r) {
                                const int row = rsub + (r & 3) + 8 * (r >> 2);
                                const bool ok = row < M;
                                const float v = ok ? keep[mi][ni][r] : 0.f;
                                float hv;
                                if (STAGED && htile) hv = (ok && cok) ? Elem<T>::to_f32(htile[(row - row_blk) * bn + (col - col_blk)]) : mu;
                                else hv = (ok && cok) ? Elem<T>::to_f32(hprev[(long)row * e.ldh + col]) : mu;
                                s1 += v; s2 = fmaf(v * (hv - mu), rstd, s2);
                            }
                        } else {
#pragma unroll
                            for (int r = 0; r < 16; ++r) {
                                const float v = (rsub + (r & 3) + 8 * (r >> 2) < M) ? keep[mi][ni][r] : 0.f;
                                s1 += v; s2 = fmaf(v, v, s2);
                            }
                        }
                    }
                    cs1[hh][ni] = s1 + __shfl_xor(s1, 32, 64);
                    cs2[hh][ni] = s2 + __shfl_xor(s2, 32, 64);
                }
            const long prow0 = (long)batch * g.tiles_m + (row_blk >> 6);
            if constexpr (MR >= 2) {
                if (lh == 0) {
#pragma unroll
                    for (int hh = 0; hh < NH; ++hh)
#pragma unroll
                        for (int ni = 0; ni < NR; ++ni) {
                            const int col = col_blk + (wn * NR + ni) * 32 + lc;
                            const long pr = prow0 + wm * NH + hh;
                            if (col < g.N && col < e.ldcs && row_blk + (wm * NH + hh) * 64 < M) {
                                cs1p[pr * e.ldcs + col] = cs1[hh][ni];
                                if (e.cs_mode != CS_SUM) cs2p[pr * e.ldcs + col] = cs2[hh][ni];
                            }
                        }
                }
            } else {
                const int wcols = NR * 32;
                __syncthreads();
                if (lh == 0) {
#pragma unroll
                    for (int ni = 0; ni < NR; ++ni) {
                        const int c = wn * wcols + ni * 32 + lc;
                        lds[(wm * 2 + 0) * bn + c] = cs1[0][ni];
                        lds[(wm * 2 + 1) * bn + c] = cs2[0][ni];
                    }
                }
                __syncthreads();
                const int t = threadIdx.x;
                if (t < bn) {
                    float s1 = 0.f, s2 = 0.f;
#pragma unroll
                    for (int w = 0; w < WM; ++w) { s1 += lds[(w * 2 + 0) * bn + t]; s2 += lds[(w * 2 + 1) * bn + t]; }
                    if (col_blk + t < g.N && col_blk + t < e.ldcs) {
                        cs1p[prow0 * e.ldcs + col_blk + t] = s1;
                        if (e.cs_mode != CS_SUM) cs2p[prow0 * e.ldcs + col_blk + t] = s2;
                    }
                }
            }
        }
        EPI_STAMP(3);
    }
#undef EPI_STAMP
}

enum { TUNE_BIT_NO_KS_GROUP = 4 };
inline bool kc_cfg_supported(int cfg) {
    return cfg == -1 || cfg == 0 || cfg == 1 || cfg == 3 || cfg == 5 || cfg == 7 || cfg == 9;
}
constexpr int KS_GROUP_MAX = 6;
struct FoldJob { const float* src; float* dst; long stride; int nsrc, n, ngroups, blocks_x; long model_stride; };
struct KsGroup {
    int n;
    int blk_end[KS_GROUP_MAX];
    FoldJob fold;
    GemmArgs g[KS_GROUP_MAX];
};

int launch_gemm_f32(int epi, const GemmArgs& g, hipStream_t s, const char** kname = nullptr);
int launch_gemm_bf16(int epi, const GemmArgs& g, hipStream_t s, const char** kname = nullptr);
int launch_gemm_fp8(int epi, const GemmArgs& g, hipStream_t s, const char** kname = nullptr);
int launch_to_fp8(const float* src, long ld_src, unsigned char* dst, long ld_dst, int rows, int cols, int prow, int pcol, float scale,
                  int transpose, hipStream_t s);
struct Quant8Args {
    const __bf16* src; long src_bs; int ld; int rows, cols, nb;
    int prow;
    unsigned char* dst; long dst_bs; int ldd;
    unsigned char* dstt; long dstt_bs; int lddt;
    Fp8Slot* slot; int fmt;
};
int launch_quant8(const Quant8Args& a, hipStream_t s);
int launch_fp8_update_scales(Fp8Slot* slots, int n, hipStream_t s);
int launch_fp8_init_slots(Fp8Slot* slots, int n, const float* targets_dev, hipStream_t s);
int launch_gemm_bf16_dw_group(const GemmArgs* gs, int n, hipStream_t s, const char** kname = nullptr,
                              const FoldJob* fold = nullptr);

constexpr int GEMM_NO_HOLES = 1 << 30;
inline GemmArgs gemm_args(int M, int N, int K, int nbatch, int tile_rows) {
    GemmArgs g;
    memset(&g, 0, sizeof g);
    g.M = M; g.N = N; g.K = K; g.nbatch = nbatch; g.splits = 1; g.kchunk = K; g.tiles_m = ceil_div(M, tile_rows);
    g.seg_stride = g.seg_rows = GEMM_NO_HOLES;
    return g;
}
inline GemmArgs gemm_fwd_args(int rows, int K, int N, int nb, const void* x, long a_bs, long lda, const void* w, long ldw,
                              bool w_transposed) {
    GemmArgs g = gemm_args(rows, N, K, nb, 64);
    g.A = x; g.a_bs = a_bs; g.a_si = lda; g.a_sk = 1;
    g.B = w;
    if (w_transposed) { g.b_sj = ldw; g.b_sk = 1; }
    else { g.b_sk = ldw; g.b_sj = 1; }
    return g;
}
inline GemmArgs gemm_dx_args(int rows, int K, int N, int nb, const void* dy, long a_bs, long ldy, const void* w, long ldw) {
    GemmArgs g = gemm_args(rows, K, N, nb, 64);
    g.A = dy; g.a_bs = a_bs; g.a_si = ldy; g.a_sk = 1;
    g.B = w; g.b_sk = 1; g.b_sj = ldw;
    return g;
}
inline int gemm_dw_kchunk(int vrows, int splits) { return (int)round_up(ceil_div(vrows, splits), 64); }
inline GemmArgs gemm_dw_args(int K, int N, int vrows, int splits, int kchunk, int seg_stride, int seg_rows, const void* x, long ldx,
                             const void* dy, long ldy, bool transposed, float* slab) {
    GemmArgs g = gemm_args(K, N, vrows, 1, 128);
    g.splits = splits; g.kchunk = kchunk;
    if (seg_stride > 0) { g.seg_stride = seg_stride; g.seg_rows = seg_rows; }
    g.A = x; g.B = dy;
    if (transposed) { g.a_si = ldx; g.a_sk = 1; g.b_sj = ldy; g.b_sk = 1; }
    else { g.a_si = 1; g.a_sk = ldx; g.b_sk = ldy; g.b_sj = 1; }
    g.e.slab = slab; g.e.slab_stride = (long)K * N; g.e.ldo = N;
    return g;
}
inline GemmArgs gemm_group(GemmArgs g, int models, long model_stride) {
    if (models <= 1) return g;
    g.e.segs = g.nbatch; g.e.model_stride = model_stride;
    g.e.model_mul = div_mul16(g.nbatch);
    g.nbatch *= models;
    return g;
}
inline int gemm_model_batches(const GemmArgs& g) { return g.e.segs > 0 ? g.e.segs : g.nbatch; }
inline int gemm_models(const GemmArgs& g) { return g.e.segs > 0 ? g.nbatch / g.e.segs : 1; }
inline long mask_pitch(int seg_rows, int ldm) { return (long)(seg_rows / 32) * ldm * 2; }

inline int epi_variant(int epi, const Epi& e) {
    if (e.act != ACT_LINEAR && e.act != ACT_RELU && e.act != ACT_SOFTPLUS) return -1;
    if (epi != EPI_FWD) return e.act;
    const bool noise = e.sigma > 0.f, mask = e.mask != nullptr;
    if (e.act == ACT_RELU ? (noise && !mask) : (mask || (noise && e.act == ACT_SOFTPLUS))) return -1;
    return e.act | (noise ? VAR_NOISE : 0) | (mask ? VAR_MASK : 0) | (noise && e.gauss ? VAR_GAUSS : 0);
}
inline int persistent_grid(int tiles, int lds_bytes) { return std::min(tiles, 256 * std::max(1, (160 * 1024) / lds_bytes)); }
template <auto KERN, int LDS, typename... Args>
int launch_with_dyn_lds(dim3 grid, dim3 block, hipStream_t s, const Args&... args) {
    static_assert(LDS <= 160 * 1024, "LDS budget of a CU");
    static DeviceOnce attr;
    if (attr.first()) {
        if (hipFuncSetAttribute((const void*)KERN, hipFuncAttributeMaxDynamicSharedMemorySize, LDS) != hipSuccess) return -2;
        attr.mark();
    }
    MRGAN_LAUNCH(KERN, grid, block, LDS, s, args...);
    return 0;
}

}
```

mr_gan_amd/csrc/gemm_bf16.hip:

```cpp
#include <algorithm>
#include <cstring>
#include <string>

#include "gemm.h"
#include "lds_ring.h"

namespace mrgan {

namespace {
constexpr int BN = 128, BK = RING_BK;
constexpr int KS_PITCH = 320;
constexpr int KS_TILE_BYTES = 64 * KS_PITCH;

#ifdef MRGAN_STAMPS
struct KcStamps { unsigned long long acc[6], prev, epi[5]; };
#define KC_STAMPS_PARAM , KcStamps& stamps_
#define KC_STAMPS_ARG , stamps_
#else
#define KC_STAMPS_PARAM
#define KC_STAMPS_ARG
#endif
template <int EPI, int BM, int BNT, int WM, int WN, int NS, int VAR>
__device__ __forceinline__ void kc_tile(const GemmArgs& g, const int batch , const int model, const int tile_m, const int tile_n, char* lds KC_STAMPS_PARAM) {
    constexpr int NW = WM * WN;
    constexpr int MR = BM / WM / 32, NR = BNT / WN / 32;
    constexpr int A_BYTES = BM * 128, B_BYTES = BNT * 128, STAGE = A_BYTES + B_BYTES;
    constexpr int A_INSTR = BM / 8 / NW, B_INSTR = BNT / 8 / NW;
    static_assert(MR >= 1 && NR >= 1 && A_INSTR >= 1 && B_INSTR >= 1 && BM % (8 * NW) == 0 && BNT % (8 * NW) == 0, "tile/wave layout");
    const int t = threadIdx.x, lane = t & 63;
    const int wave = __builtin_amdgcn_readfirstlane(t >> 6);
    const int wm = wave / WN, wn = wave % WN;
    const int lrow = lane >> 3, lp = lane & 7;
    const int lr = lane & 31, lh = lane >> 5;
    const int nk = (g.e.ablate & 4) ? 0 : g.K / BK;
#ifdef MRGAN_STAMPS
#define STAMP(i) do { const unsigned long long n_ = __builtin_amdgcn_s_memtime(); stamps_.acc[i] += n_ - stamps_.prev; stamps_.prev = n_; } while (0)
#else
#define STAMP(i)
#endif
    {
        const int row_blk = tile_m * BM, col_blk = tile_n * BNT;

        const __bf16* Ab = model_ptr((const __bf16*)g.A, g.e, model) + (long)batch * g.a_bs;
        const __bf16* Bb = model_ptr((const __bf16*)g.B, g.e, model) + (long)batch * g.b_bs;
        const __amdgpu_buffer_rsrc_t rsA = __builtin_amdgcn_make_buffer_rsrc((void*)Ab, 0, (int)((long)g.M * g.a_si * 2), 0x00020000);
        const __amdgpu_buffer_rsrc_t rsB = __builtin_amdgcn_make_buffer_rsrc((void*)Bb, 0, (int)((long)g.N * g.b_sj * 2), 0x00020000);
        int voffA[A_INSTR], voffB[B_INSTR];
#pragma unroll
        for (int i = 0; i < A_INSTR; ++i) {
            const int R = (wave * A_INSTR + i) * 8 + lrow;
            voffA[i] = (int)(((long)(row_blk + R) * g.a_si + ((lp ^ ((R >> 1) & 7)) << 3)) * 2);
        }
#pragma unroll
        for (int i = 0; i < B_INSTR; ++i) {
            const int R = (wave * B_INSTR + i) * 8 + lrow;
            voffB[i] = (int)(((long)(col_blk + R) * g.b_sj + ((lp ^ ((R >> 1) & 7)) << 3)) * 2);
        }
        auto issue = [&](int k0, int buf) {
            char* a_dst = lds + buf * STAGE + wave * A_INSTR * 1024;
            char* b_dst = lds + buf * STAGE + A_BYTES + wave * B_INSTR * 1024;
#pragma unroll
            for (int i = 0; i < A_INSTR; ++i) glds16(rsA, a_dst + i * 1024, voffA[i], k0 * 2);
#pragma unroll
            for (int i = 0; i < B_INSTR; ++i) glds16(rsB, b_dst + i * 1024, voffB[i], k0 * 2);
        };

#pragma unroll
        for (int p = 0; p < NS - 1; ++p)
            if (p < nk) issue(p * BK, p);


        const __bf16* htile = nullptr;
        if constexpr (EPI == EPI_DX && (VAR & VAR_ACT_MASK) != ACT_RELU) {
            if (dx_needs_h<VAR>(g.e)) {
                constexpr int OUTB = BM * BNT * 2 + 4 * WM * BNT * 4, RING = NS * STAGE;
                char* hdst = lds + (RING > OUTB ? RING : OUTB);
                const __bf16* hb = model_ptr((const __bf16*)g.e.h, g.e, model) + (long)batch * g.e.h_bs;
                const __amdgpu_buffer_rsrc_t rsH = __builtin_amdgcn_make_buffer_rsrc((void*)hb, 0, (int)((long)g.M * g.e.ldh * 2), 0x00020000);
                constexpr int RPI = 1024 / (BNT * 2);
                constexpr int LPR = 64 / RPI;
                constexpr int HI = BM / RPI / NW;
#pragma unroll
                for (int i = 0; i < HI; ++i) {
                    const int R = (wave * HI + i) * RPI + lane / LPR;
                    const int voff = (int)(((long)(row_blk + R) * g.e.ldh + col_blk) * 2) + (lane % LPR) * 16;
                    glds16(rsH, hdst + (wave * HI + i) * 1024, voff, 0);
// ... 80 lines not shown
__device__ __forceinline__ bf16x8 ks_frag_swz(const char* tile, int fb, int ks, int lane) {
    const int g4 = lane >> 4, i16 = lane & 15, q = i16 >> 2, p = i16 & 3;
    const int f0 = fb + (g4 & 1) * 16;
    const int m0 = ks * 16 + (g4 >> 1) * 8;
    const char* a0 = tile + (m0 + q) * 256 + ((((f0 >> 3) + (p >> 1)) ^ (q << 2)) << 4) + ((p & 1) << 3);
    const s16x4 t0 = __builtin_amdgcn_ds_read_tr16_b64_v4i16((lds_s16x4*)a0);
    const s16x4 t1 = __builtin_amdgcn_ds_read_tr16_b64_v4i16((lds_s16x4*)(a0 + 4 * 256));
    const s16x8 tt = __builtin_shufflevector(t0, t1, 0, 1, 2, 3, 4, 5, 6, 7);
    return __builtin_bit_cast(bf16x8, tt);
}

template <int NS, int WM, int WN>
__device__ __forceinline__ void ks_fast_body(const GemmArgs& g, const int bid, const int model ) {
    constexpr int NW = WM * WN;
    constexpr int MR = 128 / WM / 32, NR = 128 / WN / 32;
    constexpr int T_BYTES = 64 * 256, STAGE = 2 * T_BYTES;
    constexpr int T_INSTR = 16 / NW;
    static_assert(MR >= 1 && NR >= 1 && T_INSTR >= 1, "tile/wave layout");
    extern __shared__ __attribute__((aligned(16))) char lds[];

    const int t = threadIdx.x, lane = t & 63;
    const int wave = __builtin_amdgcn_readfirstlane(t >> 6);
    const int wm = wave / WN, wn = wave % WN;
    const int ntn = (g.N + 127) / 128, ntm = (g.M + 127) / 128;
    const int tidx = xcd_tile(bid, ntn * ntm * g.splits);
    const int split = tidx / (ntn * ntm), rem = tidx - split * (ntn * ntm);
    int tile_m, tile_n;
    if ((ntm & 7) == 0 && ntn >= 16) {
        const int grp = rem / (8 * ntn), in = rem - grp * (8 * ntn);
        tile_m = grp * 8 + (in & 7); tile_n = in >> 3;
    } else { tile_m = rem / ntn; tile_n = rem - tile_m * ntn; }
    const int row_blk = tile_m * 128, col_blk = tile_n * 128;
    const int k_begin = split * g.kchunk;
    const int k_end = (g.e.ablate & 4) ? k_begin : min(g.K, k_begin + g.kchunk);

    const __amdgpu_buffer_rsrc_t rsA = __builtin_amdgcn_make_buffer_rsrc((void*)model_ptr(g.A, g.e, model), 0, (int)((long)g.K * g.a_sk * 2), 0x00020000);
    const __amdgpu_buffer_rsrc_t rsB = __builtin_amdgcn_make_buffer_rsrc((void*)model_ptr(g.B, g.e, model), 0, (int)((long)g.K * g.b_sk * 2), 0x00020000);
    const int lrow = lane >> 4, lp = lane & 15;
    int voffA[T_INSTR], voffB[T_INSTR];
#pragma unroll
    for (int i = 0; i < T_INSTR; ++i) {
        const int kr = (wave * T_INSTR + i) * 4 + lrow;
        const int c = lp ^ ((kr & 3) << 2);
        voffA[i] = (int)(((long)kr * g.a_sk + row_blk + c * 8) * 2);
        voffB[i] = (int)(((long)kr * g.b_sk + col_blk + c * 8) * 2);
    }
    auto issue = [&](int k0, int buf) {
        char* a_dst = lds + buf * STAGE + wave * T_INSTR * 1024;
        char* b_dst = a_dst + T_BYTES;
#pragma unroll
        for (int i = 0; i < T_INSTR; ++i) glds16(rsA, a_dst + i * 1024, voffA[i], (int)((long)k0 * g.a_sk * 2));
#pragma unroll
        for (int i = 0; i < T_INSTR; ++i) glds16(rsB, b_dst + i * 1024, voffB[i], (int)((long)k0 * g.b_sk * 2));
    };

    f32x16 acc[MR][NR];
#pragma unroll
    for (int i = 0; i < MR; ++i)
#pragma unroll
        for (int j = 0; j < NR; ++j)
#pragma unroll
            for (int r = 0; r < 16; ++r) acc[i][j][r] = 0.f;

    const int nk = (k_end - k_begin + BK - 1) / BK;
#pragma unroll
    for (int p = 0; p < NS - 1; ++p)
        if (p < nk) issue(k_begin + p * BK, p);
#define KS_FRAG_A(As, mi, ks) ks_frag_swz(As, (wm * MR + mi) * 32, ks, lane)
#define KS_FRAG_B(Bs, ni, ks) ks_frag_swz(Bs, (wn * NR + ni) * 32, ks, lane)
#define KS_NO_STAMP(i)
    RING_MAINLOOP(NS, 2 * T_INSTR, MR, NR, nk, acc, issue, k_begin, KS_FRAG_A, KS_FRAG_B, lds, STAGE, T_BYTES, KS_NO_STAMP)
#undef KS_FRAG_A
#undef KS_FRAG_B
#undef KS_NO_STAMP
    __syncthreads();
    epilogue<__bf16, EPI_SLAB, MR, NR, WM>(acc, g, 0, model, split, tile_m, row_blk, col_blk, wm, wn, lane, (float*)lds, BN);
}

template <int NS, int WM, int WN>
__global__ __launch_bounds__(64 * WM * WN) void gemm_bf16_ks_fast_kernel(const GemmArgs g) {
    ks_fast_body<NS, WM, WN>(g, blockIdx.x, blockIdx.y);
}

template <int NS, int WM, int WN>
__global__ __launch_bounds__(64 * WM * WN) void gemm_bf16_ks_group_kernel(const KsGroup grp) {
    const int ngemm = grp.blk_end[grp.n - 1];
    if ((int)blockIdx.x >= ngemm) {
        const FoldJob& f = grp.fold;
        const float* fsrc = (const float*)((const char*)f.src + (long)blockIdx.y * f.model_stride);
        float* fdst = (float*)((char*)f.dst + (long)blockIdx.y * f.model_stride);
        const int fb = (int)blockIdx.x - ngemm, gidx = fb / f.blocks_x;
        const int i = (fb - gidx * f.blocks_x) * 256 + (int)threadIdx.x;
        if (threadIdx.x >= 256 || i >= f.n) return;
        float s0 = 0.f, s1 = 0.f, s2 = 0.f, s3 = 0.f;
        int p = gidx;
        for (; p + 3 * f.ngroups < f.nsrc; p += 4 * f.ngroups) {
            s0 += fsrc[(long)p * f.stride + i]; s1 += fsrc[(long)(p + f.ngroups) * f.stride + i];
            s2 += fsrc[(long)(p + 2 * f.ngroups) * f.stride + i]; s3 += fsrc[(long)(p + 3 * f.ngroups) * f.stride + i];
        }
        for (; p < f.nsrc; p += f.ngroups) s0 += fsrc[(long)p * f.stride + i];
        fdst[(long)gidx * f.stride + i] = (s0 + s1) + (s2 + s3);
        return;
    }
    int i = 0, b0 = 0;
#pragma unroll
    for (int j = 0; j < KS_GROUP_MAX - 1; ++j)
        if (j + 1 < grp.n && (int)blockIdx.x >= grp.blk_end[j]) { i = j + 1; b0 = grp.blk_end[j]; }
    ks_fast_body<NS, WM, WN>(grp.g[i], (int)blockIdx.x - b0, blockIdx.y);
}

template <int NS, int WM, int WN>
int launch_ks_fast(const GemmArgs& g, hipStream_t s) {
    static const std::string name = "gemm_bf16_ks_fast_kernel<" + std::to_string(NS) + ", " + std::to_string(WM) + ", " + std::to_string(WN) + ">";
    g_last_kernel = name.c_str();
    constexpr int STAGE = 2 * 64 * 256;
    dim3 grid(ceil_div(g.N, 128) * ceil_div(g.M, 128) * g.splits, gemm_models(g));
    return launch_with_dyn_lds<gemm_bf16_ks_fast_kernel<NS, WM, WN>, NS * STAGE>(grid, dim3(64 * WM * WN), s, g);
}

__device__ __forceinline__ bf16x8 ks_frag(const char* tile, int fb, int ks, int lane) {
    const int g4 = lane >> 4, i16 = lane & 15, q = i16 >> 2, p = i16 & 3;
    const int f0 = fb + (g4 & 1) * 16;
    const int m0 = ks * 16 + (g4 >> 1) * 8;
    const char* a0 = tile + (m0 + q) * KS_PITCH + (f0 + 4 * p) * 2;
    const s16x4 t0 = __builtin_amdgcn_ds_read_tr16_b64_v4i16((lds_s16x4*)a0);
    const s16x4 t1 = __builtin_amdgcn_ds_read_tr16_b64_v4i16((lds_s16x4*)(a0 + 4 * KS_PITCH));
    const s16x8 tt = __builtin_shufflevector(t0, t1, 0, 1, 2, 3, 4, 5, 6, 7);
    return __builtin_bit_cast(bf16x8, tt);
}

__global__ __launch_bounds__(256) void gemm_bf16_ks_kernel(const GemmArgs g) {
    __shared__ __attribute__((aligned(16))) char lds[2 * KS_TILE_BYTES];
    char* As = lds;
    char* Bs = lds + KS_TILE_BYTES;

    const int t = threadIdx.x, lane = t & 63, wave = t >> 6;
    const int wm = wave >> 1, wn = wave & 1;
    const int tile_n = blockIdx.x, tile_m = blockIdx.y;
    const int bidx = blockIdx.z / g.splits, split = blockIdx.z % g.splits;
    const int model = batch_model(g.e, bidx), batch = batch_segment(g.e, bidx, model);
    const int row_blk = tile_m * 128, col_blk = tile_n * BN;
    const int k_begin = split * g.kchunk;
    const int k_end = (g.e.ablate & 4) ? k_begin : min(g.K, k_begin + g.kchunk);

    const __bf16* A = model_ptr((const __bf16*)g.A, g.e, model) + (long)batch * g.a_bs;
    const __bf16* B = model_ptr((const __bf16*)g.B, g.e, model) + (long)batch * g.b_bs;

    f32x16 acc[2][2];
#pragma unroll
    for (int i = 0; i < 2; ++i)
#pragma unroll
        for (int j = 0; j < 2; ++j)
#pragma unroll
            for (int r = 0; r < 16; ++r) acc[i][j][r] = 0.f;

    u32x4 ra[4], rb[4];
    auto load_tile = [&](int k0) {
        const int kloc = k0 % g.seg_stride;
#pragma unroll
        for (int u = 0; u < 4; ++u) {
            const int cidx = t + 256 * u, kr = cidx >> 4, c = cidx & 15;
            const u32x4 z = {0u, 0u, 0u, 0u};
            const bool kok = (k0 + kr) < k_end && (kloc + kr) < g.seg_rows;
            ra[u] = (kok && row_blk + c * 8 < g.M) ? *(const u32x4*)(A + (long)(k0 + kr) * g.a_sk + row_blk + c * 8) : z;
            rb[u] = (kok && col_blk + c * 8 < g.N) ? *(const u32x4*)(B + (long)(k0 + kr) * g.b_sk + col_blk + c * 8) : z;
        }
    };
    auto store_tile = [&]() {
#pragma unroll
        for (int u = 0; u < 4; ++u) {
            const int cidx = t + 256 * u, kr = cidx >> 4, c = cidx & 15;
            *(u32x4*)(As + kr * KS_PITCH + c * 16) = ra[u];
            *(u32x4*)(Bs + kr * KS_PITCH + c * 16) = rb[u];
        }
    };

    if (k_begin < k_end) {
        load_tile(k_begin);
        for (int k0 = k_begin; k0 < k_end; k0 += BK) {
            __syncthreads();
            store_tile();
            __syncthreads();
            if (k0 + BK < k_end) load_tile(k0 + BK);
#pragma unroll
            for (int ks = 0; ks < BK / 16; ++ks) {
                bf16x8 a[2], b[2];
#pragma unroll
                for (int mi = 0; mi < 2; ++mi) a[mi] = ks_frag(As, (wm * 2 + mi) * 32, ks, lane);
#pragma unroll
                for (int ni = 0; ni < 2; ++ni) b[ni] = ks_frag(Bs, (wn * 2 + ni) * 32, ks, lane);
#pragma unroll
                for (int mi = 0; mi < 2; ++mi)
#pragma unroll
                    for (int ni = 0; ni < 2; ++ni)
                        acc[mi][ni] = __builtin_amdgcn_mfma_f32_32x32x16_bf16(a[mi], b[ni], acc[mi][ni], 0, 0, 0);
            }
        }
    }
    __syncthreads();
    epilogue<__bf16, EPI_SLAB, 2, 2, 2>(acc, g, batch, model, split, tile_m, row_blk, col_blk, wm, wn, lane, (float*)lds, BN);
}

__global__ void tr_probe_kernel(unsigned short* out) {
    __shared__ __attribute__((aligned(16))) unsigned short img[16 * 160];
    const int l = threadIdx.x;
    for (int i = l; i < 16 * 160; i += 64) img[i] = (unsigned short)i;
    __syncthreads();
    const s16x4 t = __builtin_amdgcn_ds_read_tr16_b64_v4i16((lds_s16x4*)((const char*)img + l * 8));
    for (int j = 0; j < 4; ++j) out[l * 8 + j] = (unsigned short)t[j];
    for (int j = 4; j < 8; ++j) out[l * 8 + j] = 0;
    __syncthreads();
    for (int i = l; i < 16 * 160; i += 64) img[i] = (unsigned short)(((i / 160) << 8) | (i % 160));
    __syncthreads();
    const s16x8 f = __builtin_bit_cast(s16x8, ks_frag((const char*)img, 0, 0, l));
    for (int j = 0; j < 8; ++j) out[512 + l * 8 + j] = (unsigned short)f[j];
}
}

template <int EPI, int VAR>
static int launch_kc_tile(const GemmArgs& g, hipStream_t s) {
    int cfg = g.e.tune_kc_cfg;
    if (cfg < 0) {
        const int nbm = gemm_model_batches(g);
        const int t128 = ceil_div(g.M, 128) * ceil_div(g.N, 128) * nbm;
        const int t256 = ceil_div(g.M, 256) * ceil_div(g.N, 256) * nbm;
        cfg = t128 >= 384 ? 7 : 0;
        if (g.K >= 2048 && t256 >= 256 && (g.N % 256) == 0) cfg = 3;
        if (EPI == EPI_FWD && cfg == 7 && g.K >= 1024 && g.K < 2048 && g.N <= 512) cfg = 5;
        if (EPI == EPI_FWD && cfg == 0 && g.K >= 1024 && g.K < 2048 && t128 >= 256 && (g.N % 128) == 0) cfg = 7;
        if (cfg == 0 && ceil_div(g.M, 64) * ceil_div(g.N, 128) * nbm <= 256) cfg = 9;
    }
    if (cfg >= 2 && cfg != 9 && (g.N % 128) != 0) cfg = 0;
    if (cfg == 3 && (g.N % 256) != 0) cfg = 1;
    constexpr bool H_TILE = EPI == EPI_DX && (VAR & VAR_ACT_MASK) != ACT_RELU;
    if (H_TILE && cfg >= 2 && cfg != 9) cfg = 1;
    if constexpr (!H_TILE) {
        if (cfg == 7) return launch_kc<EPI, 128, 128, 2, 4, 2, VAR>(g, s);
        if (cfg == 3) return launch_kc<EPI, 256, 256, 2, 4, 2, VAR>(g, s);
    }
    if (cfg == 9) return launch_kc<EPI, 64, 64, 2, 2, 3, VAR>(g, s);
    if (cfg == 1) return launch_kc<EPI, 128, 128, 2, 2, 2, VAR>(g, s);
    if (cfg == 5) return launch_kc<EPI, 64, 128, 2, 2, 2, VAR>(g, s);
    return launch_kc<EPI, 64, 128, 2, 2, 3, VAR>(g, s);
}

static int launch_kc_any(int epi, const GemmArgs& g, hipStream_t s) {
    const int var = epi_variant(epi, g.e);
    if (epi == EPI_FWD) {
        switch (var) {
            case ACT_RELU | VAR_NOISE | VAR_MASK | VAR_GAUSS: return launch_kc_tile<EPI_FWD, ACT_RELU | VAR_NOISE | VAR_MASK | VAR_GAUSS>(g, s);
            case ACT_LINEAR | VAR_NOISE | VAR_GAUSS: return launch_kc_tile<EPI_FWD, ACT_LINEAR | VAR_NOISE | VAR_GAUSS>(g, s);
            case ACT_RELU | VAR_NOISE | VAR_MASK: return launch_kc_tile<EPI_FWD, ACT_RELU | VAR_NOISE | VAR_MASK>(g, s);
            case ACT_RELU | VAR_MASK: return launch_kc_tile<EPI_FWD, ACT_RELU | VAR_MASK>(g, s);
            case ACT_RELU: return launch_kc_tile<EPI_FWD, ACT_RELU>(g, s);
            case ACT_LINEAR | VAR_NOISE: return launch_kc_tile<EPI_FWD, ACT_LINEAR | VAR_NOISE>(g, s);
            case ACT_LINEAR: return launch_kc_tile<EPI_FWD, ACT_LINEAR>(g, s);
            case ACT_SOFTPLUS: return launch_kc_tile<EPI_FWD, ACT_SOFTPLUS>(g, s);
            default: return -3;
        }
    }
    switch (var) {
        case ACT_RELU: return launch_kc_tile<EPI_DX, ACT_RELU>(g, s);
        case ACT_SOFTPLUS: return launch_kc_tile<EPI_DX, ACT_SOFTPLUS>(g, s);
        default: return launch_kc_tile<EPI_DX, ACT_LINEAR>(g, s);
    }
}

static bool ks_dense_k(const GemmArgs& g) {
    return g.a_si == 1 && g.b_sj == 1 && gemm_model_batches(g) == 1 && (g.K % BK) == 0 && (g.kchunk % BK) == 0 &&
           (g.seg_rows >= g.seg_stride || g.K <= g.seg_rows) &&
           (long)g.K * g.a_sk * 2 < (1L << 31) && (long)g.K * g.b_sk * 2 < (1L << 31);
}

int launch_gemm_bf16_dw_group(const GemmArgs* gs, int n, hipStream_t s, const char** kname, const FoldJob* fold) {
    if (n < 1 || n > KS_GROUP_MAX) return 1;
    if (gs[0].e.tune_bits & TUNE_BIT_NO_KS_GROUP) return 1;
    KsGroup grp;
    memset(&grp, 0, sizeof grp);
    grp.n = n;
    int total = 0;
    const int models = gemm_models(gs[0]);
    for (int i = 0; i < n; ++i) {
        if (!ks_dense_k(gs[i]) || gemm_models(gs[i]) != models) return 1;
        const int blocks = ceil_div(gs[i].N, 128) * ceil_div(gs[i].M, 128) * gs[i].splits;
        total += blocks;
        grp.blk_end[i] = total;
        grp.g[i] = gs[i];
    }
    if (fold && fold->n > 0) {
        grp.fold = *fold;
        grp.fold.blocks_x = ceil_div(fold->n, 256);
        total += grp.fold.blocks_x * fold->ngroups;
    }
    constexpr int STAGE = 2 * 64 * 256, LDS = 2 * STAGE;
    if (const int r = launch_with_dyn_lds<gemm_bf16_ks_group_kernel<2, 2, 4>, LDS>(dim3(total, models), dim3(512), s, grp)) return r;
    if (kname) *kname = "gemm_bf16_ks_group_kernel<2, 2, 4>";
    return hipGetLastError() == hipSuccess ? 0 : -2;
}

int launch_gemm_bf16(int epi, const GemmArgs& g, hipStream_t s, const char** kname) {
    int r = 0;
    if (epi == EPI_SLAB) {
        if (g.a_si != 1 || g.b_sj != 1) return -3;
        if (ks_dense_k(g)) {
            r = launch_ks_fast<3, 2, 4>(g, s);
        } else {
            dim3 grid(ceil_div(g.N, BN), ceil_div(g.M, 128), g.nbatch * g.splits);
            MRGAN_LAUNCH(gemm_bf16_ks_kernel, grid, dim3(256), 0, s, g);
            g_last_kernel = "gemm_bf16_ks_kernel";
        }
    } else {
        if (g.a_sk != 1 || g.b_sk != 1 || g.splits != 1 || (g.K % BK) != 0) return -3;
        if ((long)g.M * g.a_si * 2 >= (1L << 31) || (long)g.N * g.b_sj * 2 >= (1L << 31)) return -3;
        r = launch_kc_any(epi, g, s);
    }
    if (r) return r;
    if (kname) *kname = g_last_kernel;
    return hipGetLastError() == hipSuccess ? 0 : -2;
}

int launch_tr_probe(unsigned short* out, hipStream_t s) {
    MRGAN_LAUNCH(tr_probe_kernel, dim3(1), dim3(64), 0, s, out);
    return hipGetLastError() == hipSuccess ? 0 : -2;
}

}
```

mr_gan_amd/engine.py:

```python
import ctypes as C
import os

import numpy as np
import torch

_HERE = os.path.dirname(os.path.abspath(__file__))
LIB_PATH = os.path.join(_HERE, "lib", "libmrgan_hip.so")

F32, BF16, FP8 = 0, 1, 2
NET_G, NET_D = 0, 1
FLAG_SYNC_STATS, FLAG_FLAT_GRADS, FLAG_GRAPH, FLAG_GRAD_BF16, FLAG_GAUSS_NOISE = 1, 2, 4, 8, 16
NOISE_MODES = ('irwin-hall', 'gaussian')
D_GEN, D_MAIN, D_ADAM = 0, 1, 2
G_GEN, G_FEAT, G_BWD, G_TAIL, G_ADAM = 0, 1, 2, 3, 4
TUNE_CHAIN, TUNE_KC_CFG, TUNE_KS_GROUP, TUNE_PAIR_GEN, TUNE_HEAD_MFMA = 0, 1, 4, 5, 6
REGION_BN_STATS, REGION_FM_MOMENTS, REGION_BN_BWD, REGION_GRAD_D, REGION_GRAD_G, REGION_WORKSPACE = range(6)
REGION_GRAD_D_BF16, REGION_GRAD_G_BF16, REGION_TAIL_D, REGION_TAIL_G = 6, 7, 8, 9

EXPORTS = [
    "mrgan_default_config", "mrgan_workspace_bytes", "mrgan_create", "mrgan_destroy", "mrgan_last_error",
    "mrgan_num_tensors", "mrgan_tensor_shape", "mrgan_set_weights", "mrgan_get_weights", "mrgan_get_slot",
    "mrgan_set_slot", "mrgan_get_iterations", "mrgan_set_iterations", "mrgan_disc_step", "mrgan_gen_step",
    "mrgan_train_pair", "mrgan_sup_step", "mrgan_fp8_calibration", "mrgan_logmel", "mrgan_logmel_frames", "mrgan_region", "mrgan_eval_error", "mrgan_predict_logits", "mrgan_read_metrics",
    "mrgan_pair_hint", "mrgan_set_tuning", "mrgan_debug_noise", "mrgan_debug_tr_probe", "mrgan_debug_gemm_launch", "mrgan_profile_begin", "mrgan_profile_end", "mrgan_debug_ablate", "mrgan_debug_gemm_time", "mrgan_debug_buffer", "mrgan_debug_gemm_fp8",
    "mrgan_debug_quant8", "mrgan_debug_fp8_update_scales",
    "mrgan_debug_stage", "mrgan_debug_reduce_partials","mrgan_debug_colsum_finalize", "mrgan_debug_bn_apply", "mrgan_debug_bn_bwd", "mrgan_debug_head", "mrgan_debug_head_wide",
    "mrgan_debug_fm", "mrgan_debug_adam", "mrgan_debug_chain",
    "mrgan_select_model", "mrgan_sup_step_group",
    "mrgan_disc_step_group", "mrgan_gen_step_group", "mrgan_train_pair_group",
    "mrgan_input_gradient", "mrgan_attribution",
]
SAL_LOGIT, SAL_XENT, SAL_MSE = 0, 1, 2
SAL_RAW, SAL_HEATMAP = 0, 1
SAL_OBJECTIVES = {'logit': SAL_LOGIT, 'xent': SAL_XENT, 'mse': SAL_MSE}
ATTR_NOISE, ATTR_PATH = 0, 1
ATTR_MAX_DRAWS = 4096
ATTR_NOISE_SEG = 255
ATTR_METHODS = ('gradient', 'smoothgrad', 'integrated')
MAX_MODELS = 16
PROF_NAME_LEN = 96


class Config(C.Structure):
    _fields_ = [
        ("d_in", C.c_int32), ("batch", C.c_int32), ("noise_size", C.c_int32),
        ("g_hidden", C.c_int32 * 2), ("d_hidden", C.c_int32 * 5),
        ("num_classes", C.c_int32), ("dtype", C.c_int32),
        ("sigma", C.c_float * 5),
        ("lr", C.c_float), ("beta1", C.c_float), ("beta2", C.c_float), ("adam_eps", C.c_float),
        ("bn_eps", C.c_float), ("unlabeled_weight", C.c_float),
        ("seed", C.c_uint64),
        ("rank", C.c_int32), ("world", C.c_int32), ("flags", C.c_int32), ("models", C.c_int32),
    ]


class DiscArgs(C.Structure):
    _fields_ = [
        ("x_lab", C.c_void_p), ("idx_lab", C.c_void_p), ("labels", C.c_void_p),
        ("x_unl", C.c_void_p), ("idx_unl", C.c_void_p), ("z", C.c_void_p),
        ("ld_x_lab", C.c_int64), ("ld_x_unl", C.c_int64),
        ("stream_mode", C.c_int32), ("reserved", C.c_int32),
    ]


class GenArgs(C.Structure):
    _fields_ = [
        ("x_unl", C.c_void_p), ("idx_unl", C.c_void_p), ("z", C.c_void_p),
        ("ld_x_unl", C.c_int64),
        ("stream_mode", C.c_int32), ("reserved", C.c_int32),
    ]


class SupArgs(C.Structure):
    _fields_ = [
        ("x", C.c_void_p), ("idx", C.c_void_p), ("labels", C.c_void_p),
        ("ld_x", C.c_int64),
        ("stream_mode", C.c_int32), ("rows_valid", C.c_int32),
    ]


class SupGroupArgs(C.Structure):
    _fields_ = [
        ("x", C.c_void_p), ("idx", C.c_void_p), ("labels", C.c_void_p),
        ("ld_x", C.c_int64),
        ("x_model_stride", C.c_int64), ("idx_model_stride", C.c_int64), ("labels_model_stride", C.c_int64),
        ("stream_mode", C.c_int32), ("rows_valid", C.c_int32),
    ]


class DiscGroupArgs(C.Structure):
    _fields_ = [
        ("x_lab", C.c_void_p), ("idx_lab", C.c_void_p), ("labels", C.c_void_p),
        ("x_unl", C.c_void_p), ("idx_unl", C.c_void_p), ("z", C.c_void_p),
        ("ld_x_lab", C.c_int64), ("ld_x_unl", C.c_int64),
        ("x_lab_model_stride", C.c_int64), ("idx_lab_model_stride", C.c_int64), ("labels_model_stride", C.c_int64),
        ("x_unl_model_stride", C.c_int64), ("idx_unl_model_stride", C.c_int64), ("z_model_stride", C.c_int64),
        ("stream_mode", C.c_int32), ("reserved", C.c_int32),
    ]


class GenGroupArgs(C.Structure):
    _fields_ = [
        ("x_unl", C.c_void_p), ("idx_unl", C.c_void_p), ("z", C.c_void_p),
        ("ld_x_unl", C.c_int64),
        ("x_unl_model_stride", C.c_int64), ("idx_unl_model_stride", C.c_int64), ("z_model_stride", C.c_int64),
        ("stream_mode", C.c_int32), ("reserved", C.c_int32),
    ]


# ... 574 lines not shown
    ]


class DebugChainDesc(C.Structure):
    _fields_ = [
        ("variant", C.c_int32), ("fwd", DebugChainOp * 3), ("dx", DebugChainOp * 3),
        ("rows", C.c_int32), ("nseg", C.c_int32), ("block_rows", C.c_int32),
        ("models", C.c_int32), ("model_stride", C.c_int64),
        ("a", C.c_void_p), ("a_bs", C.c_int64), ("lda", C.c_int32), ("a_cols", C.c_int32),
        ("seg0", C.c_int32), ("seed", C.c_uint64), ("row0", C.c_uint32), ("gauss", C.c_int32),
        ("iter", C.c_uint32), ("batch", C.c_uint32),
        ("head", DebugHeadDesc),
        ("fm", DebugFmDesc), ("fm_feat", C.c_void_p), ("fm_ldf", C.c_int32),
    ]


class DebugAdamTile(C.Structure):
    _fields_ = [
        ("p", C.c_void_p), ("m", C.c_void_p), ("v", C.c_void_p),
        ("g", C.c_void_p), ("nslab", C.c_int32), ("slab_stride", C.c_int64),
        ("flat", C.c_void_p), ("flat16", C.c_void_p), ("w16", C.c_void_p), ("wt16", C.c_void_p),
        ("w8", C.c_void_p), ("w8t", C.c_void_p), ("w8_slot", C.c_void_p),
        ("ld", C.c_int32), ("ldt", C.c_int32), ("rows", C.c_int32), ("cols", C.c_int32),
    ]


class DebugAdamDesc(C.Structure):
    _fields_ = [
        ("tiles", C.POINTER(DebugAdamTile)), ("ntiles", C.c_int32), ("mode", C.c_int32),
        ("b1", C.c_float), ("b2", C.c_float), ("eps", C.c_float),
        ("iter", C.c_uint32), ("batch", C.c_uint32), ("lr_t", C.c_float),
        ("loss_part", C.c_void_p), ("nloss_part", C.c_int32), ("inv_rows", C.c_float), ("step_out", C.c_void_p), ("accum", C.c_void_p),
        ("flat_tail", C.c_void_p),
        ("publish_next", C.c_int32), ("advance_batch", C.c_int32), ("lr", C.c_float),
        ("models", C.c_int32), ("model_stride", C.c_int64),
    ]


def _debug_fill(d, kw):
    d._refs = []
    for name, v in kw.items():
        if isinstance(v, torch.Tensor):
            d._refs.append(v)
            v = v.data_ptr()
        elif name == "seg_kind":
            v = (C.c_int32 * 3)(*(list(v) + [0] * (3 - len(v))))
        setattr(d, name, v)
    return d


def _debug_rc(rc):
    if rc not in (0, -1, -3):
        _check(rc)
    return rc


def debug_stage(segs, **kw):
    d = _debug_fill(DebugStageDesc(), kw)
    keep = [_debug_fill(DebugStageSeg(), s) for s in segs]
    for i, s in enumerate(keep[:5]):
        d.s[i] = s
    d.nseg = len(segs)
    return _debug_rc(load_library().mrgan_debug_stage(C.byref(d), _stream()))


def debug_reduce_partials(src, nsrc, stride, n, ngroups, dst, models=1, model_stride=0):
    return _debug_rc(load_library().mrgan_debug_reduce_partials(_ptr(src), int(nsrc), C.c_int64(stride), int(n), int(ngroups), _ptr(dst),
                                                                int(models), C.c_int64(model_stride), _stream()))


def debug_colsum_finalize(part1, part2, npart, ld, n, out, nseg=1):
    return _debug_rc(load_library().mrgan_debug_colsum_finalize(_ptr(part1), _ptr(part2), int(npart), int(ld), int(n), _ptr(out), int(nseg),
                                                                _stream()))


def debug_bn_apply(**kw):
    return _debug_rc(load_library().mrgan_debug_bn_apply(C.byref(_debug_fill(DebugBnApplyDesc(), kw)), _stream()))


def debug_bn_bwd(**kw):
    return _debug_rc(load_library().mrgan_debug_bn_bwd(C.byref(_debug_fill(DebugBnBwdDesc(), kw)), _stream()))


def debug_head(**kw):
    return _debug_rc(load_library().mrgan_debug_head(C.byref(_debug_fill(DebugHeadDesc(), kw)), _stream()))


def debug_head_wide(mask=None, mask_bs=0, ldm=0, w6c=None, w6r=None, **kw):
    d = DebugHeadWideDesc()
    d.h = _debug_fill(DebugHeadDesc(), kw)
    _debug_fill(d, dict(mask=mask, mask_bs=mask_bs, ldm=ldm, w6c=w6c, w6r=w6r))
    return _debug_rc(load_library().mrgan_debug_head_wide(C.byref(d), _stream()))


def debug_fm(**kw):
    return _debug_rc(load_library().mrgan_debug_fm(C.byref(_debug_fill(DebugFmDesc(), kw)), _stream()))


CH_V_DTAIL, CH_V_GFWD, CH_V_GBWD = range(3)


def debug_chain(fwd=(), dx=(), head=None, fm=None, **kw):
    d = _debug_fill(DebugChainDesc(), kw)
    keep = [d._refs]
    for name, ops in (("fwd", fwd), ("dx", dx)):
        for i, o in enumerate(list(ops)[:3]):
            op = _debug_fill(DebugChainOp(), o)
            keep.append(op._refs)
            getattr(d, name)[i] = op
    if head is not None:
        h = _debug_fill(DebugHeadDesc(), head)
        keep.append(h._refs)
        d.head = h
    if fm is not None:
        f = _debug_fill(DebugFmDesc(), fm)
        keep.append(f._refs)
        d.fm = f
    name = C.create_string_buffer(PROF_NAME_LEN)
    stream = _stream() if torch.cuda.is_available() else None
    rc = _debug_rc(load_library().mrgan_debug_chain(C.byref(d), name, PROF_NAME_LEN, stream))
    del keep
    return rc, name.value.decode()


def debug_adam(tiles, **kw):
    arr = (DebugAdamTile * len(tiles))(*[_debug_fill(DebugAdamTile(), t) for t in tiles])
    d = _debug_fill(DebugAdamDesc(), kw)
    d.tiles, d.ntiles = arr, len(tiles)
    nxt = (C.c_uint32 * 4)()
    rc = _debug_rc(load_library().mrgan_debug_adam(C.byref(d), nxt, _stream()))
    return rc, (np.array(list(nxt), dtype=np.uint32) if d.publish_next and rc == 0 else None)


def debug_gemm(dtype, op, a, b, bias=None, act=0, splits=1):
    td = torch.bfloat16 if dtype == BF16 else torch.float32
    m = a.shape[0]
    k, n = (a.shape[1], b.shape[1]) if op == 2 else b.shape
    if n % 64 or k % 64:
        raise ValueError("debug_gemm: n and k must be multiples of 64")
    a, b = a.to(td).contiguous(), b.to(td).contiguous()
    if op == 0:
        wt = dtype == BF16
        out = torch.zeros((m, n), dtype=td, device=a.device)
        d = debug_gemm_desc(dtype=dtype, op=0, m=m, n=n, k=k, a=a, a_si=k, a_sk=1, b=b.t().contiguous() if wt else b,
                            b_sk=1 if wt else n, b_sj=k if wt else 1, act=act, n_valid=n, bias=bias, out=out, ldo=n)
    elif op == 1:
        out = torch.zeros((m, k), dtype=td, device=a.device)
        d = debug_gemm_desc(dtype=dtype, op=1, m=m, n=k, k=n, a=a, a_si=n, a_sk=1, b=b, b_sk=1, b_sj=n, n_valid=k, out=out, ldo=k)
    else:
        splits = max(1, splits)
        out = torch.zeros((splits, k, n), dtype=torch.float32, device=a.device)
        d = debug_gemm_desc(dtype=dtype, op=2, m=k, n=n, k=m, splits=splits, kchunk=-(-(-(-m // splits)) // 64) * 64,
                            a=a, a_si=1, a_sk=k, b=b, b_sk=n, b_sj=1, slab=out, slab_stride=k * n, ldo=n)
    _check(debug_gemm_launch(d)[0])
    for s in range(1, splits if op == 2 else 0):
        out[0] += out[s]
    return out[0] if op == 2 else out.float()


def fp8_slots(rows, device="cuda:0"):
    return torch.from_numpy(np.array(rows, dtype=np.float32).reshape(-1, 4).view(np.int32)).to(device)


def fp8_slots_read(slots):
    w = slots.cpu().numpy()
    return w[:, 0].view(np.uint32).copy(), w[:, 1:].copy().view(np.float32)
# ... 36 lines not shown
```

Baseline: 2592 steps/s.

## Fuse generator BatchNorm backward into grouped weight-gradient GEMM producer

Instead of a separate BatchNorm-backward kernel writing dpre1g and then a grouped weight-gradient GEMM reading it, the first-layer generator dW job now computes the BN backward elementwise while staging its B operand in LDS. It also writes the db partials per 64-row chunk. Separately, when not folding, the first layer's split-K slabs can reuse the dpre1g buffer so it can take more splits. This removes one kernel launch and a full round trip of the activation gradient through memory. In exchange each fused block recomputes the column-stat folds and carries extra LDS.

```diff
diff --git a/include/mrgan_abi.h b/include/mrgan_abi.h
--- a/include/mrgan_abi.h
+++ b/include/mrgan_abi.h
@@ -131,7 +131,8 @@
     MRGAN_TUNE_KC_CFG = 1,
     MRGAN_TUNE_KS_GROUP = 4,
     MRGAN_TUNE_PAIR_GEN = 5,
-    MRGAN_TUNE_HEAD_MFMA = 6
+    MRGAN_TUNE_HEAD_MFMA = 6,
+    MRGAN_TUNE_BN_FOLD = 7
 };
 int mrgan_set_tuning(mrgan_handle* h, int knob, int value);
 
diff --git a/include/mrgan_debug.h b/include/mrgan_debug.h
--- a/include/mrgan_debug.h
+++ b/include/mrgan_debug.h
@@ -93,6 +93,9 @@
     float* db_part;
 } mrgan_debug_bn_bwd_desc;
 int mrgan_debug_bn_bwd(const mrgan_debug_bn_bwd_desc* d, mrgan_stream stream);
+int mrgan_debug_bn_fold_launch(const mrgan_debug_gemm_desc* d, const mrgan_debug_bn_bwd_desc* bn, int models, int64_t model_stride,
+                               char* kname, int kname_len, mrgan_stream stream);
+int mrgan_debug_bn_fold_applies(int dtype, int flags, int batch, int noise_size, int ks_group, int bn_fold);
 
 typedef struct mrgan_debug_head_desc {
     int32_t dtype;
diff --git a/mr_gan_amd/csrc/aux_kernels.h b/mr_gan_amd/csrc/aux_kernels.h
--- a/mr_gan_amd/csrc/aux_kernels.h
+++ b/mr_gan_amd/csrc/aux_kernels.h
@@ -50,6 +50,60 @@
 };
 int launch_bn_bwd(int bf16, const BnBwdArgs& a, hipStream_t s);
 int stat_row_blocks(int rows);
+
+constexpr int STAT_CB = 64;
+template <int NT, int NA>
+__device__ __forceinline__ void fold_partials_n(const float* const (&part)[NA], int npart, int ldcs, int col0, int ncols, float (*scr)[STAT_CB],
+                                                float* const (&out)[NA]) {
+    constexpr int G = NT / 256;
+    const int t = threadIdx.x, grp = G > 1 ? t >> 8 : 0, tl = G > 1 ? t & 255 : t;
+    const int cq = (tl & 15) * 4, pl = tl >> 4, c0 = col0 + grp * STAT_CB;
+    f32x4 s0[NA], s1[NA];
+#pragma unroll
+    for (int a = 0; a < NA; ++a) { s0[a] = f32x4{0.f, 0.f, 0.f, 0.f}; s1[a] = s0[a]; }
+    if (c0 + cq < ncols) {
+        int p = pl;
+        for (; p + 16 < npart; p += 32) {
+#pragma unroll
+            for (int a = 0; a < NA; ++a) {
+                s0[a] += *(const f32x4*)(part[a] + (long)p * ldcs + c0 + cq);
+                s1[a] += *(const f32x4*)(part[a] + (long)(p + 16) * ldcs + c0 + cq);
+            }
+        }
+        for (; p < npart; p += 16) {
+#pragma unroll
+            for (int a = 0; a < NA; ++a) s0[a] += *(const f32x4*)(part[a] + (long)p * ldcs + c0 + cq);
+        }
+    }
+#pragma unroll
+    for (int a = 0; a < NA; ++a) {
+        s0[a] += s1[a];
+        *(f32x4*)(&scr[(a * G + grp) * 16 + pl][cq]) = s0[a];
+    }
+    __syncthreads();
+    if (tl < STAT_CB) {
+#pragma unroll
+        for (int a = 0; a < NA; ++a) {
+            float s = 0.f;
+#pragma unroll
+            for (int k = 0; k < 16; ++k) s += scr[(a * G + grp) * 16 + k][tl];
+            out[a][grp * STAT_CB + tl] = s;
+        }
+    }
+    __syncthreads();
+}
+__device__ __forceinline__ void fold_partials(const float* part, int npart, int ldcs, int col0, int ncols, float (*scr)[STAT_CB], float* out) {
+    const float* const p[1] = {part};
+    float* const o[1] = {out};
+    fold_partials_n<256, 1>(p, npart, ldcs, col0, ncols, scr, o);
+}
+__device__ __forceinline__ float bn_bwd_elem(float hv, float d, float count, float cA, float cB, float cM, float cR, float cG, float& acc) {
+    const float xh = (hv - cM) * cR;
+    const float dh = cA * (count * d - cB - xh * cG);
+    const float o = dh * (-expm1f(-hv));
+    acc += o;
+    return o;
+}
 
 enum { HEAD_LAB = 0, HEAD_UNL = 1, HEAD_FAKE = 2, HEAD_EVAL = 3, HEAD_LOGITS = 4,
        HEAD_MSE = 5,
diff --git a/mr_gan_amd/csrc/aux_kernels.hip b/mr_gan_amd/csrc/aux_kernels.hip
--- a/mr_gan_amd/csrc/aux_kernels.hip
+++ b/mr_gan_amd/csrc/aux_kernels.hip
@@ -127,30 +127,7 @@
     }
 }
 
-constexpr int RB = 64, CB = 64;
-
-__device__ __forceinline__ void fold_partials(const float* part, int npart, int ldcs, int col0, int ncols, float (*scr)[CB], float* out) {
-    const int t = threadIdx.x, cq = (t & 15) * 4, pl = t >> 4;
-    f32x4 s0 = {0.f, 0.f, 0.f, 0.f}, s1 = s0;
-    if (col0 + cq < ncols) {
-        int p = pl;
-        for (; p + 16 < npart; p += 32) {
-            s0 += *(const f32x4*)(part + (long)p * ldcs + col0 + cq);
-            s1 += *(const f32x4*)(part + (long)(p + 16) * ldcs + col0 + cq);
-        }
-        for (; p < npart; p += 16) s0 += *(const f32x4*)(part + (long)p * ldcs + col0 + cq);
-    }
-    s0 += s1;
-    *(f32x4*)(&scr[pl][cq]) = s0;
-    __syncthreads();
-    if (t < CB) {
-        float s = 0.f;
-#pragma unroll
-        for (int k = 0; k < 16; ++k) s += scr[k][t];
-        out[t] = s;
-    }
-    __syncthreads();
-}
+constexpr int RB = 64, CB = STAT_CB;
 
 template <typename T>
 __global__ __launch_bounds__(256) void bn_apply_kernel(const BnApplyArgs a) {
@@ -226,10 +203,7 @@
 #pragma unroll
             for (int i = 0; i < 8; ++i) {
                 const int c = cg * 8 + i;
-                const float xh = (hv[i] - cM[c]) * cR[c];
-                const float dh = cA[c] * (a.count * d[i] - cB[c] - xh * cG[c]);
-                o[i] = dh * (-expm1f(-hv[i]));
-                acc[i] += o[i];
+                o[i] = bn_bwd_elem(hv[i], d[i], a.count, cA[c], cB[c], cM[c], cR[c], cG[c], acc[i]);
             }
             store8<T>(dpre + (long)r * a.ld + c0, o);
         }
diff --git a/mr_gan_amd/csrc/engine.hip b/mr_gan_amd/csrc/engine.hip
--- a/mr_gan_amd/csrc/engine.hip
+++ b/mr_gan_amd/csrc/engine.hip
@@ -183,22 +183,24 @@
 
 struct DwJob { const Dense* L; const void* x; const void* dy; };
 
-int dense_dw_all(mrgan_handle* h, int kind, const DwJob* jobs, int n, int rows, int nseg, hipStream_t s, const FoldJob* fold = nullptr) {
+int dense_dw_all(mrgan_handle* h, int kind, const DwJob* jobs, int n, int rows, int nseg, hipStream_t s, const FoldJob* fold = nullptr,
+                 const BnFoldJob* bnf = nullptr) {
     GemmArgs gs[KS_GROUP_MAX];
     DwJob js[KS_GROUP_MAX];
     double fl[KS_GROUP_MAX], total = 0.0, bytes = 0.0;
     if (n > KS_GROUP_MAX) return fail(-1, "dense_dw_all: too many products");
     std::copy(jobs, jobs + n, js);
     const int ngroup = (int)(std::stable_partition(js, js + n, [](const DwJob& j) { return !j.L->q.on; }) - js);
+    if (bnf && (!h->bf16 || ngroup != n)) return fail(-1, "dense_dw_all: the BatchNorm-backward job needs the grouped launch");
     for (int i = 0; i < n; ++i) fl[i] = dw_args(h, gs[i], *js[i].L, kind, js[i].x, js[i].dy, rows, nseg);
     for (int i = 0; i < ngroup; ++i) { total += fl[i] * h->grouped; bytes += dw_bytes(h, (double)rows * nseg, *js[i].L) * h->grouped; }
     int first = 0;
     if (h->bf16 && ngroup > 0) {
         const char* kname = "gemm";
         prof_arm(h);
-        const int r = launch_gemm_bf16_dw_group(gs, ngroup, s, &kname, fold);
+        const int r = launch_gemm_bf16_dw_group(gs, ngroup, s, &kname, fold, bnf);
         prof_done(h, kname, total, bytes);
-        if (r < 0) return fail(r, "grouped weight-gradient launch failed");
+        if (r < 0 || (r && bnf)) return fail(r < 0 ? r : -1, "grouped weight-gradient launch failed");
         if (r == 0) { first = ngroup; fold = nullptr; }
     }
     for (int i = first; i < n; ++i) CHK(run_gemm(h, EPI_SLAB, gs[i], fl[i], dw_bytes(h, (double)rows * nseg, *js[i].L), s));
@@ -577,9 +579,25 @@
         b.ldcs = N1p; b.count = h->stat_count; b.gamma = h->gt[2].p; b.mu = h->bn_mu; b.rstd = h->bn_rstd;
         b.db_part = h->db1g_part;
         b.models = h->grouped; b.model_stride = (long)h->W;
-        PROF("bn_bwd_kernel", launch_bn_bwd(h->bf16, b, s));
         const DwJob jobs[3] = {{&h->g[2], h->h2, h->dxfake}, {&h->g[0], h->zbuf, h->dpre1g}, {&h->g[1], h->hbn, h->dpre2g}};
-        CHK(dense_dw_all(h, KIND_G, jobs, 3, B, 1, s));
+        if (bn_fold_applies(h->bf16, h->fp8, h->flat_grads, B, h->nzp, h->tune_bits)) {
+            BnFoldJob f;
+            memset(&f, 0, sizeof f);
+            f.on = 1; f.job = 1;
+            f.dy = b.dy; f.h = b.h; f.ld = b.ld; f.rows = b.rows; f.cols = b.cols;
+            f.cs1 = b.cs1; f.cs2 = b.cs2; f.npart = b.npart; f.ldcs = b.ldcs; f.count = b.count;
+            f.gamma = b.gamma; f.mu = b.mu; f.rstd = b.rstd; f.db_part = b.db_part;
+            f.model_stride = h->grouped > 1 ? (long)h->W : 0;
+            CHK(dense_dw_all(h, KIND_G, jobs, 3, B, 1, s, nullptr, &f));
+        } else if (h->g1_slabs_in_dpre1g) {
+            b.dpre = h->dhbn;
+            PROF("bn_bwd_kernel", launch_bn_bwd(h->bf16, b, s));
+            const DwJob inplace[3] = {jobs[0], {&h->g[0], h->zbuf, h->dhbn}, jobs[2]};
+            CHK(dense_dw_all(h, KIND_G, inplace, 3, B, 1, s));
+        } else {
+            PROF("bn_bwd_kernel", launch_bn_bwd(h->bf16, b, s));
+            CHK(dense_dw_all(h, KIND_G, jobs, 3, B, 1, s));
+        }
         if (h->flat_grads) CHK(run_adam(h, MRGAN_NET_G, ADAM_REDUCE_ONLY, false, s));
     } else if (phase == MRGAN_G_ADAM) {
         CHK(run_adam(h, MRGAN_NET_G, h->flat_grads ? ADAM_FROM_FLAT : ADAM_FUSED, false, s, a->stream_mode ? 1 : 0));
diff --git a/mr_gan_amd/csrc/engine_debug.hip b/mr_gan_amd/csrc/engine_debug.hip
--- a/mr_gan_amd/csrc/engine_debug.hip
+++ b/mr_gan_amd/csrc/engine_debug.hip
@@ -415,6 +415,51 @@
     return debug_finish("debug_bn_bwd", launch_bn_bwd(d->dtype == MRGAN_BF16, a, s), s);
 }
 
+int mrgan_debug_bn_fold_launch(const mrgan_debug_gemm_desc* d, const mrgan_debug_bn_bwd_desc* bn, int models, int64_t model_stride,
+                               char* kname, int kname_len, mrgan_stream stream) {
+    if (!d || !bn) return fail(-1, "debug_bn_fold_launch: null argument");
+    if (kname && kname_len > 0) kname[0] = 0;
+    if (d->dtype != MRGAN_BF16 || bn->dtype != MRGAN_BF16 || d->op != 2) return fail(-1, "debug_bn_fold_launch: a bf16 weight gradient");
+    if (models < 1 || (models > 1 && (model_stride <= 0 || (model_stride % 16)))) return fail(-1, "debug_bn_fold_launch: models >= 1, model_stride a multiple of 16 bytes");
+    if (!bn->dy || !bn->h || !bn->gamma || !bn->mu || !bn->rstd || !bn->db_part || bn->rows < 1 || bn->cols < 1) return fail(-1, "debug_bn_fold_launch: null argument");
+    if (int r = debug_cs_check("debug_bn_fold_launch", bn->cs1, bn->cs2, bn->npart, bn->ldcs, bn->ld)) return r;
+    if (bn->ld < bn->cols || (bn->ld % 8) || !al(bn->h, 16) || !al(bn->dy, 16)) return fail(-1, "debug_bn_fold_launch: ld >= cols, ld %% 8 == 0 and 16-byte aligned dy / h");
+    if (d->m > 128 || d->n > bn->ld || bn->rows > d->k) return fail(-1, "debug_bn_fold_launch: one 128-row output tile, n <= ld, rows <= k");
+    hipStream_t s = (hipStream_t)stream;
+    DevState* st = nullptr;
+    if (int r = debug_devstate(d->iter, 0, 0.f, &st)) return r;
+    GemmArgs g;
+    int epi = 0;
+    mrgan_debug_gemm_desc dd = *d;
+    if (!dd.b) { dd.b = bn->dy; dd.b_sk = bn->ld; dd.b_sj = 1; }
+    int r = debug_gemm_args(dd, st, g, epi);
+    const char* name = "";
+    if (!r) {
+        g = gemm_group(g, models, (long)model_stride);
+        BnFoldJob f;
+        memset(&f, 0, sizeof f);
+        f.on = 1; f.job = 0;
+        f.dy = bn->dy; f.h = bn->h; f.ld = bn->ld; f.rows = bn->rows; f.cols = bn->cols;
+        f.cs1 = bn->cs1; f.cs2 = bn->cs2; f.npart = bn->npart; f.ldcs = bn->ldcs; f.count = bn->count;
+        f.gamma = bn->gamma; f.mu = bn->mu; f.rstd = bn->rstd; f.db_part = bn->db_part;
+        f.model_stride = models > 1 ? (long)model_stride : 0;
+        r = launch_gemm_bf16_dw_group(&g, 1, s, &name, nullptr, &f);
+        if (r) r = fail(r < 0 ? r : -3, "debug_bn_fold_launch: launch refused (%d)", r);
+    }
+    const hipError_t he = hipStreamSynchronize(s);
+    hipFree(st);
+    if (!r && he != hipSuccess) return fail(-10, "debug_bn_fold_launch: %s", hipGetErrorString(he));
+    if (!r && kname && kname_len > 0) snprintf(kname, (size_t)kname_len, "%s", name);
+    return r;
+}
+
+int mrgan_debug_bn_fold_applies(int dtype, int flags, int batch, int noise_size, int ks_group, int bn_fold) {
+    const bool fp8 = dtype == MRGAN_FP8;
+    const int padw = fp8 ? 128 : 64;
+    const int bits = (ks_group ? 0 : TUNE_BIT_NO_KS_GROUP) | (bn_fold ? 0 : TUNE_BIT_NO_BN_FOLD);
+    return bn_fold_applies(dtype == MRGAN_BF16 || fp8, fp8, (flags & MRGAN_FLAG_FLAT_GRADS) != 0, batch, (int)round_up(noise_size, padw), bits) ? 1 : 0;
+}
+
 int mrgan_debug_head(const mrgan_debug_head_desc* d, mrgan_stream stream) {
     if (!d || !d->f || !d->w || !d->b || d->rows < 1 || d->nseg < 1 || d->nseg > 3 || d->feat < 1 || d->classes < 1) return fail(-1, "debug_head: null argument");
     if (d->dtype != MRGAN_F32 && d->dtype != MRGAN_BF16) return fail(-1, "debug_head: dtype must be fp32 or bf16");
diff --git a/mr_gan_amd/csrc/engine_internal.h b/mr_gan_amd/csrc/engine_internal.h
--- a/mr_gan_amd/csrc/engine_internal.h
+++ b/mr_gan_amd/csrc/engine_internal.h
@@ -112,6 +112,7 @@
     float *head_part, *head_red, *loss_part; int head_stride, head_groups;
     int head_nblk;
     int bnb_blocks;
+    bool g1_slabs_in_dpre1g;
     bool fp8; int fp8_cal[2];
     Fp8Slot* slots; float* slot_targets; float* accum_save;
     float* fm_scratch; unsigned int* fm_count;
@@ -140,4 +141,15 @@
 int fp8_refresh_weights(mrgan_handle* h, int net, hipStream_t s);
 int fp8_update_scales(mrgan_handle* h, hipStream_t s);
 
+inline bool bn_fold_applies(bool bf16, bool fp8, bool flat_grads, int batch, int nz_pad, int tune_bits) {
+    return bf16 && !fp8 && !flat_grads && batch > 0 && (batch % 64) == 0 && nz_pad <= 128 &&
+           (tune_bits & (TUNE_BIT_NO_KS_GROUP | TUNE_BIT_NO_BN_FOLD)) == 0;
 }
+#ifndef MRGAN_BN_FOLD_TILES
+#define MRGAN_BN_FOLD_TILES 4
+#endif
+inline int bn_fold_splits(int splits, int vrows, int max_slabs) {
+    return std::max(splits, std::min(max_slabs, vrows / (64 * MRGAN_BN_FOLD_TILES)));
+}
+
+}
diff --git a/mr_gan_amd/csrc/engine_state.hip b/mr_gan_amd/csrc/engine_state.hip
--- a/mr_gan_amd/csrc/engine_state.hip
+++ b/mr_gan_amd/csrc/engine_state.hip
@@ -247,6 +247,13 @@
         Dense& L = h->g[l];
         L.splits = (h->fp8 && l == 1) ? 1 : splits_g;
         L.slabs = a.take<float>((size_t)L.splits * L.Kp * L.Np);
+        if (l == 0) h->g1_slabs_in_dpre1g = false;
+        if (l == 0 && bn_fold_applies(h->bf16, h->fp8, h->flat_grads, B, h->nzp, 0)) {
+            const int fs = bn_fold_splits(splits_g, S, MAX_SLABS);
+            if (fs > splits_g && (size_t)fs * L.Kp * L.Np * sizeof(float) <= (size_t)S * N1p * es) {
+                L.splits = fs; L.slabs = (float*)h->dpre1g; h->g1_slabs_in_dpre1g = true;
+            }
+        }
     }
     auto src = [&](Tensor& t, const float* g, int nslab, long stride) { t.g = g; t.nslab = nslab; t.slab_stride = stride; };
     for (int l = 0; l < 5; ++l) src(*h->d[l].W, h->d[l].slabs, h->d[l].splits, (long)h->d[l].Kp * h->d[l].Np);
@@ -506,6 +513,7 @@
         case MRGAN_TUNE_KS_GROUP: h->tune_bits = (h->tune_bits & ~TUNE_BIT_NO_KS_GROUP) | (value ? 0 : TUNE_BIT_NO_KS_GROUP); break;
         case MRGAN_TUNE_PAIR_GEN: h->tune_pair_gen = value ? 1 : 0; break;
         case MRGAN_TUNE_HEAD_MFMA: h->head_wide = value != 0 && h->head_wide_ok; break;
+        case MRGAN_TUNE_BN_FOLD: h->tune_bits = (h->tune_bits & ~TUNE_BIT_NO_BN_FOLD) | (value ? 0 : TUNE_BIT_NO_BN_FOLD); break;
         default: return fail(-1, "unknown tuning knob %d", knob);
     }
     return 0;
diff --git a/mr_gan_amd/csrc/gemm.h b/mr_gan_amd/csrc/gemm.h
--- a/mr_gan_amd/csrc/gemm.h
+++ b/mr_gan_amd/csrc/gemm.h
@@ -394,16 +394,26 @@
 #undef EPI_STAMP
 }
 
-enum { TUNE_BIT_NO_KS_GROUP = 4 };
+enum { TUNE_BIT_NO_KS_GROUP = 4, TUNE_BIT_NO_BN_FOLD = 8 };
 inline bool kc_cfg_supported(int cfg) {
     return cfg == -1 || cfg == 0 || cfg == 1 || cfg == 3 || cfg == 5 || cfg == 7 || cfg == 9;
 }
 constexpr int KS_GROUP_MAX = 6;
 struct FoldJob { const float* src; float* dst; long stride; int nsrc, n, ngroups, blocks_x; long model_stride; };
+struct BnFoldJob {
+    int on, job;
+    const void* dy; const void* h; int ld, rows, cols;
+    const float* cs1; const float* cs2; int npart, ldcs;
+    float count;
+    const float* gamma; const float* mu; const float* rstd;
+    float* db_part;
+    long model_stride;
+};
 struct KsGroup {
     int n;
     int blk_end[KS_GROUP_MAX];
     FoldJob fold;
+    BnFoldJob bnf;
     GemmArgs g[KS_GROUP_MAX];
 };
 
@@ -423,7 +433,7 @@
 int launch_fp8_update_scales(Fp8Slot* slots, int n, hipStream_t s);
 int launch_fp8_init_slots(Fp8Slot* slots, int n, const float* targets_dev, hipStream_t s);
 int launch_gemm_bf16_dw_group(const GemmArgs* gs, int n, hipStream_t s, const char** kname = nullptr,
-                              const FoldJob* fold = nullptr);
+                              const FoldJob* fold = nullptr, const BnFoldJob* bnf = nullptr);
 
 constexpr int GEMM_NO_HOLES = 1 << 30;
 inline GemmArgs gemm_args(int M, int N, int K, int nbatch, int tile_rows) {
diff --git a/mr_gan_amd/csrc/gemm_bf16.hip b/mr_gan_amd/csrc/gemm_bf16.hip
--- a/mr_gan_amd/csrc/gemm_bf16.hip
+++ b/mr_gan_amd/csrc/gemm_bf16.hip
@@ -2,6 +2,7 @@
 #include <cstring>
 #include <string>
 
+#include "aux_kernels.h"
 #include "gemm.h"
 #include "lds_ring.h"
 
@@ -248,6 +249,137 @@
     ks_fast_body<NS, WM, WN>(g, blockIdx.x, blockIdx.y);
 }
 
+constexpr int KS_BNF_CONST_BYTES = 5 * 128 * 4;
+template <int WM, int WN>
+__device__ __forceinline__ void ks_bnfold_body(const GemmArgs& g, const BnFoldJob& f, const int bid, const int model) {
+    constexpr int NW = WM * WN;
+    constexpr int MR = 128 / WM / 32, NR = 128 / WN / 32;
+    constexpr int T_BYTES = 64 * 256, STAGE = 2 * T_BYTES;
+    constexpr int T_INSTR = 16 / NW;
+    static_assert(NW == 8 && MR == 2 && NR == 1, "512 threads: two 16-byte chunks of a 64 x 128 k-tile each");
+    extern __shared__ __attribute__((aligned(16))) char lds[];
+    char* const Bimg = lds + T_BYTES;
+    float (*const red)[128] = (float (*)[128])(lds + STAGE + T_BYTES);
+    float* const cA = (float*)(lds + 2 * STAGE);
+    float* const cB = cA + 128; float* const cM = cA + 256; float* const cR = cA + 384; float* const cG = cA + 512;
+
+    const int t = threadIdx.x, lane = t & 63;
+    const int wave = __builtin_amdgcn_readfirstlane(t >> 6);
+    const int wm = wave / WN, wn = wave % WN;
+    const int ntn = (g.N + 127) / 128, ntm = (g.M + 127) / 128;
+    const int tidx = xcd_tile(bid, ntn * ntm * g.splits);
+    const int split = tidx / (ntn * ntm), rem = tidx - split * (ntn * ntm);
+    const int tile_m = rem / ntn, tile_n = rem - tile_m * ntn;
+    const int row_blk = tile_m * 128, col_blk = tile_n * 128;
+    const int k_begin = split * g.kchunk;
+    const int k_end = (g.e.ablate & 4) ? k_begin : min(g.K, k_begin + g.kchunk);
+    const int nk = k_end > k_begin ? (k_end - k_begin) / BK : 0;
+
+    const __amdgpu_buffer_rsrc_t rsA = __builtin_amdgcn_make_buffer_rsrc((void*)model_ptr(g.A, g.e, model), 0, (int)((long)g.K * g.a_sk * 2), 0x00020000);
+    const int lrow = lane >> 4, lp = lane & 15;
+    int voffA[T_INSTR];
+#pragma unroll
+    for (int i = 0; i < T_INSTR; ++i) {
+        const int kr = (wave * T_INSTR + i) * 4 + lrow;
+        voffA[i] = (int)(((long)kr * g.a_sk + row_blk + (lp ^ ((kr & 3) << 2)) * 8) * 2);
+    }
+    auto issue_a = [&](int k0, int buf) {
+        char* a_dst = lds + buf * STAGE + wave * T_INSTR * 1024;
+#pragma unroll
+        for (int i = 0; i < T_INSTR; ++i) glds16(rsA, a_dst + i * 1024, voffA[i], (int)((long)k0 * g.a_sk * 2));
+    };
+
+    const long moff = (long)model * f.model_stride;
+    const __bf16* const dy = (const __bf16*)((const char*)f.dy + moff);
+    const __bf16* const hh = (const __bf16*)((const char*)f.h + moff);
+    const int cg = t & 15, rl = t >> 4, c0 = col_blk + cg * 8;
+    const bool col_ok = c0 < f.ld && c0 < g.N;
+    u32x4 rd[2], rh[2];
+    auto load_b = [&](int k0, int u) {
+        const long off = (long)min(k0 + rl + 32 * u, f.rows - 1) * f.ld + (col_ok ? c0 : 0);
+        rd[u] = *(const u32x4*)(dy + off);
+        rh[u] = *(const u32x4*)(hh + off);
+    };
+
+    f32x16 acc[MR][NR];
+#pragma unroll
+    for (int i = 0; i < MR; ++i)
+#pragma unroll
+        for (int r = 0; r < 16; ++r) acc[i][0][r] = 0.f;
+
+    if (nk > 0) {
+        issue_a(k_begin, 0);
+        load_b(k_begin, 0); load_b(k_begin, 1);
+        float gm = 0.f, mu = 0.f, rs = 0.f;
+        if (t < 128 && col_blk + t < f.cols) {
+            const int col = col_blk + t;
+            gm = ((const float*)((const char*)f.gamma + moff))[col]; mu = ((const float*)((const char*)f.mu + moff))[col];
+            rs = ((const float*)((const char*)f.rstd + moff))[col];
+        }
+        const float* const parts[2] = {(const float*)((const char*)f.cs1 + moff), (const float*)((const char*)f.cs2 + moff)};
+        float* const outs[2] = {cB, cG};
+        fold_partials_n<64 * NW, 2>(parts, f.npart, f.ldcs, col_blk, f.ld, (float (*)[STAT_CB])red, outs);
+        if (t < 128) { cA[t] = gm * rs / f.count; cM[t] = mu; cR[t] = rs; }
+    }
+    float* const db = (float*)((char*)f.db_part + moff);
+    int buf = 0;
+    for (int kt = 0; kt < nk; ++kt) {
+        const int k0 = k_begin + kt * BK;
+        asm volatile("s_waitcnt vmcnt(0) lgkmcnt(0)" ::: "memory");
+        __builtin_amdgcn_s_barrier();
+        asm volatile("" ::: "memory");
+        float bsum[8];
+#pragma unroll
+        for (int i = 0; i < 8; ++i) bsum[i] = 0.f;
+#pragma unroll
+        for (int u = 0; u < 2; ++u) {
+            const int kr = rl + 32 * u;
+            bf16x8 o8;
+#pragma unroll
+            for (int i = 0; i < 8; ++i) o8[i] = (__bf16)0.f;
+            if (col_ok && k0 + kr < f.rows) {
+                const bf16x8 h8 = __builtin_bit_cast(bf16x8, rh[u]), d8 = __builtin_bit_cast(bf16x8, rd[u]);
+#pragma unroll
+                for (int i = 0; i < 8; ++i) {
+                    const int c = cg * 8 + i;
+                    o8[i] = (__bf16)bn_bwd_elem((float)h8[i], (float)d8[i], f.count, cA[c], cB[c], cM[c], cR[c], cG[c], bsum[i]);
+                }
+            }
+            *(bf16x8*)(Bimg + kr * 256 + ((cg ^ ((kr & 3) << 2)) << 4)) = o8;
+            if (kt + 1 < nk) load_b(k0 + BK, u);
+        }
+#pragma unroll
+        for (int i = 0; i < 8; i += 4) *(f32x4*)&red[rl][cg * 8 + i] = f32x4{bsum[i], bsum[i + 1], bsum[i + 2], bsum[i + 3]};
+        if (kt + 1 < nk) issue_a(k0 + BK, buf ^ 1);
+        asm volatile("s_waitcnt lgkmcnt(0)" ::: "memory");
+        __builtin_amdgcn_s_barrier();
+        asm volatile("" ::: "memory");
+        const char* As = lds + buf * STAGE;
+        buf ^= 1;
+        bf16x8 a[4][MR], b[4];
+#pragma unroll
+        for (int kk = 0; kk < 4; ++kk) {
+#pragma unroll
+            for (int mi = 0; mi < MR; ++mi) a[kk][mi] = ks_frag_swz(As, (wm * MR + mi) * 32, kk, lane);
+            b[kk] = ks_frag_swz(Bimg, wn * 32, kk, lane);
+        }
+        __builtin_amdgcn_sched_barrier(0);
+#pragma unroll
+        for (int kk = 0; kk < 4; ++kk)
+#pragma unroll
+            for (int mi = 0; mi < MR; ++mi)
+                acc[mi][0] = __builtin_amdgcn_mfma_f32_32x32x16_bf16(a[kk][mi], b[kk], acc[mi][0], 0, 0, 0);
+        if (t < 128 && col_blk + t < f.ld && k0 < f.rows) {
+            float s = 0.f;
+#pragma unroll
+            for (int k = 0; k < 32; ++k) s += red[k][t];
+            db[(long)(k0 >> 6) * f.ld + col_blk + t] = s;
+        }
+    }
+    __syncthreads();
+    epilogue<__bf16, EPI_SLAB, MR, NR, WM>(acc, g, 0, model, split, tile_m, row_blk, col_blk, wm, wn, lane, (float*)lds, BN);
+}
+
 template <int NS, int WM, int WN>
 __global__ __launch_bounds__(64 * WM * WN) void gemm_bf16_ks_group_kernel(const KsGroup grp) {
     const int ngemm = grp.blk_end[grp.n - 1];
@@ -272,6 +404,11 @@
 #pragma unroll
     for (int j = 0; j < KS_GROUP_MAX - 1; ++j)
         if (j + 1 < grp.n && (int)blockIdx.x >= grp.blk_end[j]) { i = j + 1; b0 = grp.blk_end[j]; }
+    if (grp.bnf.on && i == grp.bnf.job) {
+        static_assert(NS == 2, "ks_bnfold_body lays its images over a 2-stage ring");
+        ks_bnfold_body<WM, WN>(grp.g[i], grp.bnf, (int)blockIdx.x - b0, blockIdx.y);
+        return;
+    }
     ks_fast_body<NS, WM, WN>(grp.g[i], (int)blockIdx.x - b0, blockIdx.y);
 }
 
@@ -438,9 +575,20 @@
            (long)g.K * g.a_sk * 2 < (1L << 31) && (long)g.K * g.b_sk * 2 < (1L << 31);
 }
 
-int launch_gemm_bf16_dw_group(const GemmArgs* gs, int n, hipStream_t s, const char** kname, const FoldJob* fold) {
+static bool bn_fold_job_ok(const GemmArgs* gs, int n, const BnFoldJob& f) {
+    if (f.job < 0 || f.job >= n) return false;
+    const GemmArgs& g = gs[f.job];
+    if (!f.dy || !f.h || !f.cs1 || !f.cs2 || !f.gamma || !f.mu || !f.rstd || !f.db_part) return false;
+    if (g.M > 128 || g.N > f.ld || (f.ld % 8) || f.cols < 1 || f.cols > f.ld || f.rows < 1 || f.rows > g.K) return false;
+    if (f.npart < 1 || (f.ldcs % 4) || f.ldcs < f.ld || !(f.count > 0.f)) return false;
+    return ((uintptr_t)f.dy % 16) == 0 && ((uintptr_t)f.h % 16) == 0 && ((uintptr_t)f.cs1 % 16) == 0 && ((uintptr_t)f.cs2 % 16) == 0 &&
+           (f.model_stride % 16) == 0;
+}
+
+int launch_gemm_bf16_dw_group(const GemmArgs* gs, int n, hipStream_t s, const char** kname, const FoldJob* fold, const BnFoldJob* bnf) {
     if (n < 1 || n > KS_GROUP_MAX) return 1;
     if (gs[0].e.tune_bits & TUNE_BIT_NO_KS_GROUP) return 1;
+    if (bnf && bnf->on && !bn_fold_job_ok(gs, n, *bnf)) return -3;
     KsGroup grp;
     memset(&grp, 0, sizeof grp);
     grp.n = n;
@@ -458,7 +606,8 @@
         grp.fold.blocks_x = ceil_div(fold->n, 256);
         total += grp.fold.blocks_x * fold->ngroups;
     }
-    constexpr int STAGE = 2 * 64 * 256, LDS = 2 * STAGE;
+    if (bnf && bnf->on) grp.bnf = *bnf;
+    constexpr int STAGE = 2 * 64 * 256, LDS = 2 * STAGE + KS_BNF_CONST_BYTES;
     if (const int r = launch_with_dyn_lds<gemm_bf16_ks_group_kernel<2, 2, 4>, LDS>(dim3(total, models), dim3(512), s, grp)) return r;
     if (kname) *kname = "gemm_bf16_ks_group_kernel<2, 2, 4>";
     return hipGetLastError() == hipSuccess ? 0 : -2;
diff --git a/mr_gan_amd/engine.py b/mr_gan_amd/engine.py
--- a/mr_gan_amd/engine.py
+++ b/mr_gan_amd/engine.py
@@ -13,7 +13,7 @@
 NOISE_MODES = ('irwin-hall', 'gaussian')
 D_GEN, D_MAIN, D_ADAM = 0, 1, 2
 G_GEN, G_FEAT, G_BWD, G_TAIL, G_ADAM = 0, 1, 2, 3, 4
-TUNE_CHAIN, TUNE_KC_CFG, TUNE_KS_GROUP, TUNE_PAIR_GEN, TUNE_HEAD_MFMA = 0, 1, 4, 5, 6
+TUNE_CHAIN, TUNE_KC_CFG, TUNE_KS_GROUP, TUNE_PAIR_GEN, TUNE_HEAD_MFMA, TUNE_BN_FOLD = 0, 1, 4, 5, 6, 7
 REGION_BN_STATS, REGION_FM_MOMENTS, REGION_BN_BWD, REGION_GRAD_D, REGION_GRAD_G, REGION_WORKSPACE = range(6)
 REGION_GRAD_D_BF16, REGION_GRAD_G_BF16, REGION_TAIL_D, REGION_TAIL_G = 6, 7, 8, 9
 
@@ -24,7 +24,7 @@
     "mrgan_train_pair", "mrgan_sup_step", "mrgan_fp8_calibration", "mrgan_logmel", "mrgan_logmel_frames", "mrgan_region", "mrgan_eval_error", "mrgan_predict_logits", "mrgan_read_metrics",
     "mrgan_pair_hint", "mrgan_set_tuning", "mrgan_debug_noise", "mrgan_debug_tr_probe", "mrgan_debug_gemm_launch", "mrgan_profile_begin", "mrgan_profile_end", "mrgan_debug_ablate", "mrgan_debug_gemm_time", "mrgan_debug_buffer", "mrgan_debug_gemm_fp8",
     "mrgan_debug_quant8", "mrgan_debug_fp8_update_scales",
-    "mrgan_debug_stage", "mrgan_debug_reduce_partials","mrgan_debug_colsum_finalize", "mrgan_debug_bn_apply", "mrgan_debug_bn_bwd", "mrgan_debug_head", "mrgan_debug_head_wide",
+    "mrgan_debug_stage", "mrgan_debug_reduce_partials","mrgan_debug_colsum_finalize", "mrgan_debug_bn_apply", "mrgan_debug_bn_bwd", "mrgan_debug_bn_fold_launch", "mrgan_debug_bn_fold_applies", "mrgan_debug_head", "mrgan_debug_head_wide",
     "mrgan_debug_fm", "mrgan_debug_adam", "mrgan_debug_chain",
     "mrgan_select_model", "mrgan_sup_step_group",
     "mrgan_disc_step_group", "mrgan_gen_step_group", "mrgan_train_pair_group",
@@ -765,6 +765,17 @@
     return _debug_rc(load_library().mrgan_debug_bn_bwd(C.byref(_debug_fill(DebugBnBwdDesc(), kw)), _stream()))
 
 
+def debug_bn_fold_launch(desc, models=1, model_stride=0, **bn):
+    name = C.create_string_buffer(PROF_NAME_LEN)
+    rc = _debug_rc(load_library().mrgan_debug_bn_fold_launch(C.byref(desc), C.byref(_debug_fill(DebugBnBwdDesc(), bn)), int(models),
+                                                             C.c_int64(model_stride), name, PROF_NAME_LEN, _stream()))
+    return rc, name.value.decode()
+
+
+def bn_fold_applies(dtype, flags, batch, noise_size=100, ks_group=1, bn_fold=1):
+    return bool(load_library().mrgan_debug_bn_fold_applies(int(dtype), int(flags), int(batch), int(noise_size), int(ks_group), int(bn_fold)))
+
+
 def debug_head(**kw):
     return _debug_rc(load_library().mrgan_debug_head(C.byref(_debug_fill(DebugHeadDesc(), kw)), _stream()))
 
```

Result: no change. 2625 steps/s, median of 4 (+1.3%).
